# apple/ml-mdm

Measured on AMD Instinct MI355X. Metric: denoise-steps/sec, whole job = N x optimizer steps/s at per-GPU batch 64 (train fwd+bwd+optimizer, cc12m_64x64 U-Net), higher is better.
Workload: dtype bf16; 1 GPU; unet64 train step, per-GPU batch 64, global batch 64; global_batch=64, parallelism=dp1, settle_steps=15

## Files before the change

### include/mdm_hip_ext.h

```cpp
#ifndef MDM_HIP_EXT_H_
#define MDM_HIP_EXT_H_
#ifdef __cplusplus
extern "C" {
#endif

int mdm_attn_cross_bias(const void* qkv, const void* kvc, const float* mask, const float* bias, int bias_ld,
                        const void* base, int base_ld, void* out, int B, int L, int S, int H, int d, int dtype,
                        void* stream);

int mdm_freeu_plan(int N, int H, int W, int C1, int C2, int dtype, int structure, size_t* ws_bytes);
int mdm_freeu_stats(const void* h, const void* r, void* ws, size_t ws_bytes, int N, int H, int W, int C1, int C2,
                    int structure, int dtype, void* stream);
int mdm_freeu_apply(const void* h, const void* r, const void* ws, size_t ws_bytes, void* out, int N, int H, int W, int C1,
                    int C2, float b, float s, int structure, int dtype, void* stream);

int mdm_cfg_plan(int B, size_t chw, int rescale_on, size_t* ws_bytes);
int mdm_cfg_stats(const float* x_t, const float* pred, const float* pred_uncond, const float* gamma, const float* run_prev,
                  float* run_out, const float* run_gate, const float* w_gate, float momentum, int rescale_on, void* ws,
                  size_t ws_bytes, int B, size_t chw, int pred_type, void* stream);
int mdm_cfg_combine(const float* x_t, const float* pred, const float* pred_uncond, const float* gamma, const float* run,
                    const float* w_gate, const void* ws, size_t ws_bytes, float* out, float guidance, float eta,
                    float norm_threshold, float rescale, float image_scale, int B, size_t chw, int pred_type, void* stream);

int mdm_tiles_gather(const float* x, float* out, int B, int C, int H, int W, int h, int w, int sy, int sx, int reps,
                     void* stream);
int mdm_tiles_merge(const float* p, float* out, int R, int C, int H, int W, int h, int w, int sy, int sx, int blend,
                    void* stream);

int mdm_abs_quantile_plan(int B, size_t n, size_t* ws_bytes);
int mdm_abs_quantile(const float* x, void* ws, size_t ws_bytes, int B, size_t n, float q, float cmin, float cmax, float* thr,
                     float* stats, void* stream);

int mdm_t5_attn_fwd_lse(const void* qkv, const int* seq_start, const int* pos, const float* bias_table, void* out, float* lse,
                        int B, int T, int S, int max_len, int H, int d, int dtype, void* stream);
int mdm_t5_attn_bwd(const void* qkv, const void* out, const float* lse, const void* dout, const int* seq_start, const int* pos,
                    const float* bias_table, void* dqkv, int B, int T, int S, int max_len, int H, int d, int dtype,
                    void* stream);
int mdm_t5_gated_gelu_bwd(const void* u, const void* dy, void* du, int T, int F, int dtype, void* stream);
int mdm_t5_rms_bwd(const float* x, const float* ln_w, const void* dh, float* dx, void* dx_lo, int T, int D, float eps,
                   int dtype, void* stream);
int mdm_t5_final_rms_bwd(const float* x, const void* delta, const float* ln_w, const float* dout, const int* flat, float* dx,
                         void* dx_lo, int T, int D, float eps, int dtype, void* stream);
int mdm_t5_embed_rms_slots(const int* ids, const float* table, const int* slot_of_id, const float* learned, const float* ln_w,
                           float* x, void* h, int T, int D, int vocab, int n_ids, int P, float eps, int dtype, void* stream);
int mdm_t5_embed_bwd(const float* dx0, const int* slot_start, const int* tokens, float* dlearned, int P, int D, int n, int T,
                     void* stream);

int mdm_sampler_step_sa(const float* x_t, const float* pred, const float* pred_uncond, float guidance, const float* gamma,
                        const float* gamma_last, const float* gamma_h0, const float* gamma_h1, const float* gate,
                        const float* thr, const float* noise, const unsigned long long* rng_state, int rng_stream, float* h0,
                        float* h1, float* psum, float* x0_out, float* x_last_out, int B, size_t chw, int pred_type, int clip,
                        float image_scale, int max_predictor, int max_corrector, void* stream);

#ifdef __cplusplus
}
#endif
#endif
```

### ml-mdm_amd/csrc/gemm_conv.hip

```cpp
#include <stdio.h>
#include <stdlib.h>

#include <type_traits>
#include <utility>

#include "common.hpp"
#include "conv_args.hpp"

namespace mdm {



__device__ __forceinline__ void load4(const float* p, float (&o)[4]) {
  const f32x4 t = *reinterpret_cast<const f32x4*>(p);
  o[0] = t[0]; o[1] = t[1]; o[2] = t[2]; o[3] = t[3];
}
__device__ __forceinline__ void load4(const bf16* p, float (&o)[4]) {
  const bf16x4 t = *reinterpret_cast<const bf16x4*>(p);
  o[0] = (float)t[0]; o[1] = (float)t[1]; o[2] = (float)t[2]; o[3] = (float)t[3];
}

__device__ __attribute__((aligned(16))) uint4 g_zero_page[4] = {};


// ... 1165 lines not shown
#define MDM_BLDS(rs, lds_off, voff, soff)                                                                   \
  __builtin_amdgcn_raw_ptr_buffer_load_lds(rs, (__attribute__((address_space(3))) void*)(lds_off), 16, voff, soff, 0, 0)
#define MDM_WG_TILE_STATE(it_)                                                                              \
  const bool more_ = (it_) < nt;                                                                            \
  const auto rsA = __builtin_amdgcn_make_buffer_rsrc(a_base, 0, more_ ? a_bytes : 0u, 0x00020000);         \
  const auto rsB = __builtin_amdgcn_make_buffer_rsrc(b_base, 0, more_ ? b_bytes : 0u, 0x00020000);         \
  const int mb_ = (mt_begin + (it_)) * BKM;                                                                 \
  const int a_soff = mb_ * p.Cout * 2, b_soff = mb_ * p.Cin * 2;
#define MDM_WG_PIECE(stage, q)                                                                              \
  {                                                                                                         \
    constexpr int j_ = (q) >> 1;                                                                            \
    const int m_ = mb_ + j_ * RPP + srow;                                                                   \
    bool v_ = m_ < p.M;                                                                                     \
    if (((q) & 1) == 0) {                                                                                   \
      MDM_BLDS(rsA, (stage) + j_ * (RPP * ROWB) + wave_lds, v_ ? a_vo[j_] : INVALID, a_soff);               \
    } else {                                                                                                \
      if (MODE == MODE_3x3) {                                                                               \
        const int ow_ = m_ & (p.W - 1), oh_ = (m_ >> logW) & (p.H - 1);                                     \
        v_ = v_ && (unsigned)(oh_ + kh - 1) < (unsigned)p.H && (unsigned)(ow_ + kw - 1) < (unsigned)p.W;    \
      }                                                                                                     \
      MDM_BLDS(rsB, (stage) + A_BYTES + j_ * (RPP * ROWB) + wave_lds, v_ ? b_vo[j_] : INVALID, b_soff);     \
    }                                                                                                       \
  }

  f32x4 acc[MT][NT];
#pragma unroll
  for (int i = 0; i < MT; ++i)
#pragma unroll
    for (int j = 0; j < NT; ++j) acc[i][j] = f32x4{0.f, 0.f, 0.f, 0.f};
  const int bias_k0 = (MODE == MODE_3x3 && p.skip_cout > 0) ? (((n0 / p.skip_cout) >> 1) * 3 + ((n0 / p.skip_cout) & 1)) * p.Cin : 0;
  constexpr int BR = MT / NWN;
  const int wn_s = __builtin_amdgcn_readfirstlane(wn);
  const int bias_share = p.groups > 0 ? 1 : p.bias_share;
  const int kt_rel = k0 >= bias_k0 ? (k0 - bias_k0) / BN : bias_share;
  const bool bias_blk = (p.groups > 0 ? gr.bout[grp] != nullptr : p.bslab != nullptr) && kt_rel < bias_share;
  const int bias_chunk = (nt + bias_share - 1) / bias_share;
  const int bias_b0 = bias_blk ? min(kt_rel * bias_chunk, nt) : nt;
  const int bias_b1 = bias_blk ? min(bias_b0 + bias_chunk, nt) : nt;

  unsigned fa[MT], fb[NT];
  {
    const unsigned smem_base = (unsigned)(size_t)(__attribute__((address_space(3))) char*)smem;
    const int r0 = quad * 8 + (l16 >> 2);
    const int fsw = (l16 >> 2) | ((quad & 1) << 2);
#pragma unroll
    for (int c = 0; c < MT; ++c) fa[c] = smem_base + r0 * ROWB + (((wm * MT + c) ^ fsw) << 5) + ((l16 & 3) << 3);
#pragma unroll
    for (int c = 0; c < NT; ++c) fb[c] = smem_base + A_BYTES + r0 * ROWB + (((wn * NT + c) ^ fsw) << 5) + ((l16 & 3) << 3);
  }

  if (nt > 0) {
    {
      MDM_WG_TILE_STATE(0);
      MDM_WG_PIECE(smem, 0); MDM_WG_PIECE(smem, 1); MDM_WG_PIECE(smem, 2); MDM_WG_PIECE(smem, 3);
      MDM_WG_PIECE(smem, 4); MDM_WG_PIECE(smem, 5); MDM_WG_PIECE(smem, 6); MDM_WG_PIECE(smem, 7);
    }
    {
      MDM_WG_TILE_STATE(1);
      MDM_WG_PIECE(smem + STAGE, 0); MDM_WG_PIECE(smem + STAGE, 1); MDM_WG_PIECE(smem + STAGE, 2); MDM_WG_PIECE(smem + STAGE, 3);
      MDM_WG_PIECE(smem + STAGE, 4); MDM_WG_PIECE(smem + STAGE, 5); MDM_WG_PIECE(smem + STAGE, 6); MDM_WG_PIECE(smem + STAGE, 7);
    }
    asm volatile("s_waitcnt vmcnt(0)" ::: "memory");
    __syncthreads();
    u32x2 ra[MT][2], rb0[NT][2], rb1[NT][2];
#pragma unroll
    for (int c = 0; c < NT; ++c) MDM_TR2(rb0[c][0], rb0[c][1], fb[c], 0);
#pragma unroll
    for (int c = 0; c < MT; ++c) MDM_TR2(ra[c][0], ra[c][1], fa[c], 0);
    __builtin_amdgcn_sched_barrier(0);

#define MDM_WG_ITER(BIAS)                                                                                   \
    {                                                                                                       \
      const unsigned so = (unsigned)((it & 1) * STAGE), sn = (unsigned)(((it + 1) & 1) * STAGE);            \
                                                                     \
      _Pragma("unroll") for (int c = 0; c < NT; ++c) { const unsigned ad = fb[c] + so; MDM_TR2(rb1[c][0], rb1[c][1], ad, KS1); } \
      Frag<T> bq[NT];                                                                                       \
      _Pragma("unroll") for (int i = 0; i < MT; ++i) {                                                      \
        if (i == 0) {                                                                                       \
          asm volatile("s_waitcnt lgkmcnt(%8)"                                                              \
                       : "+v"(rb0[0][0]), "+v"(rb0[0][1]), "+v"(rb0[1][0]), "+v"(rb0[1][1]), "+v"(rb0[2][0]), \
                         "+v"(rb0[2][1]), "+v"(rb0[3][0]), "+v"(rb0[3][1])                                  \
                       : "n"(WAITN) : "memory");                                                            \
          _Pragma("unroll") for (int j = 0; j < NT; ++j) bq[j] = frag_of(rb0[j][0], rb0[j][1]);             \
        }                                                                                                   \
        asm volatile("s_waitcnt lgkmcnt(%2)" : "+v"(ra[i][0]), "+v"(ra[i][1]) : "n"(WAITN) : "memory");     \
        const Frag<T> aq = frag_of(ra[i][0], ra[i][1]);                                                     \
        _Pragma("unroll") for (int j = 0; j < NT; ++j) mma16(acc[i][j], bq[j], aq);                         \
        if (BIAS && i / BR == wn_s) bsum[i % BR] = frag_sum_guarded(aq, bsum[i % BR]);                      \
        { const unsigned ad = fa[i] + so; MDM_TR2(ra[i][0], ra[i][1], ad, KS1); }                           \
        __builtin_amdgcn_sched_barrier(0);                                                                  \
      }                                                                                                     \
                                        \
      asm volatile("s_waitcnt vmcnt(0) lgkmcnt(0)" ::: "memory");                                           \
      __builtin_amdgcn_s_barrier();                                                                         \
      __builtin_amdgcn_sched_barrier(0);                                                                    \
              \
      MDM_WG_TILE_STATE(it + 2);                                                                            \
      char* const dst = smem + so;                                                                          \
      _Pragma("unroll") for (int c = 0; c < NT; ++c) { const unsigned ad = fb[c] + sn; MDM_TR2(rb0[c][0], rb0[c][1], ad, 0); } \
      _Pragma("unroll") for (int j = 0; j < NT; ++j) bq[j] = frag_of(rb1[j][0], rb1[j][1]);                 \
      _Pragma("unroll") for (int i = 0; i < MT; ++i) {                                                      \
        const Frag<T> aq = frag_of(ra[i][0], ra[i][1]);                                                     \
        _Pragma("unroll") for (int j = 0; j < NT; ++j) mma16(acc[i][j], bq[j], aq);                         \
        if (BIAS && i / BR == wn_s) bsum[i % BR] = frag_sum_guarded(aq, bsum[i % BR]);                      \
        if (MT == 8) { MDM_WG_PIECE_RT(dst, i) } else { MDM_WG_PIECE_RT(dst, 2 * i) MDM_WG_PIECE_RT(dst, 2 * i + 1) } \
        { const unsigned ad = fa[i] + sn; MDM_TR2(ra[i][0], ra[i][1], ad, 0); }                             \
        __builtin_amdgcn_sched_barrier(0);                                                                  \
      }                                                                                                     \
    }
#define MDM_WG_PIECE_RT(stage, q)                                                                           \
    switch (q) {                                                                                            \
      case 0: MDM_WG_PIECE(stage, 0) break; case 1: MDM_WG_PIECE(stage, 1) break;                           \
      case 2: MDM_WG_PIECE(stage, 2) break; case 3: MDM_WG_PIECE(stage, 3) break;                           \
      case 4: MDM_WG_PIECE(stage, 4) break; case 5: MDM_WG_PIECE(stage, 5) break;                           \
      case 6: MDM_WG_PIECE(stage, 6) break; default: MDM_WG_PIECE(stage, 7) break;                          \
    }
    int it = 0;
    float bsum[BR];
    for (; it < bias_b0; ++it) MDM_WG_ITER(false)
#pragma unroll
    for (int i = 0; i < BR; ++i) bsum[i] = 0.f;
    for (; it < bias_b1; ++it) MDM_WG_ITER(true)
    if (bias_blk) {
#pragma unroll
      for (int r = 0; r < BR; ++r) {
        float v = bsum[r];
        v += __shfl_xor(v, 16, 64);
        v += __shfl_xor(v, 32, 64);
        const int n = n0 + wm * TM + (wn * BR + r) * 16 + l16;
        if (quad == 0 && n < p.Cout) {
          if (p.groups > 0) gr.bout[grp][n] += v;
          else p.bslab[((size_t)split * bias_share + kt_rel) * p.Cout + n] = v;
        }
      }
    }
    for (; it < nt; ++it) MDM_WG_ITER(false)
    asm volatile("s_waitcnt vmcnt(0) lgkmcnt(0)" ::: "memory");
#undef MDM_WG_PIECE_RT
#undef MDM_WG_ITER
  } else if (bias_blk && p.groups == 0 && quad == 0) {
#pragma unroll
    for (int r = 0; r < BR; ++r) {
      const int n = n0 + wm * TM + (wn * BR + r) * 16 + l16;
      if (n < p.Cout) p.bslab[((size_t)split * bias_share + kt_rel) * p.Cout + n] = 0.f;
    }
  }
#undef MDM_WG_PIECE
#undef MDM_WG_TILE_STATE
#undef MDM_BLDS

  if (bias_blk && p.groups == 0 && split == 0 && kt_rel == 0 && n0 == 0 && tid == 0)
    reinterpret_cast<int*>(p.bslab - WG_BHDR)[0] = bias_share;
  const bool direct = p.groups > 0;
  float* __restrict__ S = direct ? gr.out[grp] : p.slab + (size_t)split * p.Cout * p.K;
  const bool vec_ok = (p.K & 3) == 0;
  if (!direct) {
#pragma unroll
    for (int i = 0; i < MT; ++i) {
      const int n = n0 + wm * TM + i * 16 + l16;
      if (n >= p.Cout) continue;
#pragma unroll
      for (int j = 0; j < NT; ++j) {
        const int k = k0 + wn * TN + j * 16 + quad * 4;
        if (k >= p.K) continue;
        float* o = S + (size_t)n * p.K + k;
        if (vec_ok) {
          *reinterpret_cast<f32x4*>(o) = acc[i][j];
        } else {
#pragma unroll
          for (int e = 0; e < 4; ++e) if (k + e < p.K) o[e] = acc[i][j][e];
        }
      }
    }
  } else if (vec_ok && n0 + BM <= p.Cout && k0 + BN <= p.K) {
    float* const o0 = S + (size_t)(n0 + wm * TM + l16) * p.K + k0 + wn * TN + quad * 4;
    f32x4 old[2][NT];
#pragma unroll
    for (int j = 0; j < NT; ++j) old[0][j] = *reinterpret_cast<const f32x4*>(o0 + j * 16);
#pragma unroll
    for (int i = 0; i < MT; ++i) {
      if (i + 1 < MT) {
#pragma unroll
        for (int j = 0; j < NT; ++j) old[(i + 1) & 1][j] = *reinterpret_cast<const f32x4*>(o0 + (size_t)(i + 1) * 16 * p.K + j * 16);
      }
#pragma unroll
      for (int j = 0; j < NT; ++j) *reinterpret_cast<f32x4*>(o0 + (size_t)i * 16 * p.K + j * 16) = old[i & 1][j] + acc[i][j];
    }
  } else {
#pragma unroll
    for (int i = 0; i < MT; ++i) {
      const int n = n0 + wm * TM + i * 16 + l16;
      if (n >= p.Cout) continue;
#pragma unroll
      for (int j = 0; j < NT; ++j) {
        const int k = k0 + wn * TN + j * 16 + quad * 4;
        if (k >= p.K) continue;
        float* o = S + (size_t)n * p.K + k;
#pragma unroll
        for (int e = 0; e < 4; ++e) if (k + e < p.K) o[e] += acc[i][j][e];
      }
    }
  }
#endif
}
#undef MDM_TR2

template <int NT>
__device__ __forceinline__ void wgrad_bias_reduce(const float* __restrict__ bslab, float* __restrict__ dbias, int splits,
                                                  int Cout, int accumulate, int blk, float* lds) {
  constexpr int G = NT / 32;
  const int tid = threadIdx.x, c = tid & 31, g = tid >> 5;
  const int rows = splits * reinterpret_cast<const int*>(bslab - WG_BHDR)[0];
  const int o = blk * 32 + c;
  float s0 = 0.f, s1 = 0.f, s2 = 0.f, s3 = 0.f;
  if (o < Cout) {
    const float* src = bslab + o;
    int r = g;
    for (; r + 3 * G < rows; r += 4 * G) {
      s0 += src[(size_t)r * Cout];
      s1 += src[(size_t)(r + G) * Cout];
      s2 += src[(size_t)(r + 2 * G) * Cout];
      s3 += src[(size_t)(r + 3 * G) * Cout];
    }
    for (; r < rows; r += G) s0 += src[(size_t)r * Cout];
  }
  lds[tid] = (s0 + s1) + (s2 + s3);
  __syncthreads();
  if (g == 0 && o < Cout) {
    float s = lds[c];
#pragma unroll
    for (int q = 1; q < G; ++q) s += lds[q * 32 + c];
    dbias[o] = accumulate ? dbias[o] + s : s;
  }
}

__global__ __launch_bounds__(192) void wgrad_reduce_kernel(const float* __restrict__ slab, float* __restrict__ dw,
                                                           const float* __restrict__ bslab, float* __restrict__ dbias,
                                                           int splits, int Cout, int Cin, int taps, int accumulate,
                                                           int bblocks) {
  __shared__ float tile[64 * 9 + 4];
  const int tid = threadIdx.x;
  if ((int)blockIdx.x < bblocks) {
    wgrad_bias_reduce<192>(bslab, dbias, splits, Cout, accumulate, (int)blockIdx.x, tile);
    return;
  }
  const int wb = (int)blockIdx.x - bblocks;
  const int iblocks = (Cin + 63) / 64;
  const int o = wb / iblocks, i0 = (wb - o * iblocks) * 64;
  const int ni = min(64, Cin - i0);
  const size_t total = (size_t)Cout * Cin * taps;
  const int K = Cin * taps;
  const int per_o = taps * 16;
  if (tid < per_o) {
    const int tp = tid >> 4, i4 = (tid & 15) * 4;
    f32x4 acc[8];
#pragma unroll
    for (int u = 0; u < 8; ++u) acc[u] = f32x4{0.f, 0.f, 0.f, 0.f};
    if (i4 < ni) {
      const float* src = slab + (size_t)o * K + (size_t)tp * Cin + i0 + i4;
      int sp = 0;
      for (; sp + 8 <= splits; sp += 8) {
#pragma unroll
        for (int u = 0; u < 8; ++u) acc[u] += *reinterpret_cast<const f32x4*>(src + (size_t)(sp + u) * total);
      }
      for (; sp < splits; ++sp) acc[0] += *reinterpret_cast<const f32x4*>(src + (size_t)sp * total);
    }
    const f32x4 s4 = ((acc[0] + acc[1]) + (acc[2] + acc[3])) + ((acc[4] + acc[5]) + (acc[6] + acc[7]));
#pragma unroll
    for (int q = 0; q < 4; ++q) tile[(i4 + q) * taps + tp] = s4[q];
  }
  __syncthreads();
  const int run = ni * taps;
  float* const dst = dw + ((size_t)o * Cin + i0) * taps;
  for (int r = tid; r < run; r += 192) dst[r] = accumulate ? dst[r] + tile[r] : tile[r];
}

__global__ __launch_bounds__(256) void wgrad_reduce_flat_kernel(const float* __restrict__ slab, float* __restrict__ dw,
                                                                const float* __restrict__ bslab,
                                                                float* __restrict__ dbias, int splits, int Cout,
                                                                size_t total, int accumulate, int wblocks, int bblocks) {
  if ((int)blockIdx.x < bblocks) {
    __shared__ float part[256];
    wgrad_bias_reduce<256>(bslab, dbias, splits, Cout, accumulate, (int)blockIdx.x, part);
    return;
  }
  const size_t n4 = total / 4;
  const f32x4* s4 = reinterpret_cast<const f32x4*>(slab);
  f32x4* d4 = reinterpret_cast<f32x4*>(dw);
  for (size_t i = (size_t)(blockIdx.x - bblocks) * 256 + threadIdx.x; i < n4; i += (size_t)wblocks * 256) {
    f32x4 a0 = s4[i], a1 = {0.f, 0.f, 0.f, 0.f}, a2 = a1, a3 = a1;
    int sp = 1;
    for (; sp + 4 <= splits; sp += 4) {
      a0 += s4[(size_t)sp * n4 + i];
      a1 += s4[(size_t)(sp + 1) * n4 + i];
      a2 += s4[(size_t)(sp + 2) * n4 + i];
      a3 += s4[(size_t)(sp + 3) * n4 + i];
    }
    for (; sp < splits; ++sp) a0 += s4[(size_t)sp * n4 + i];
    const f32x4 a = (a0 + a1) + (a2 + a3);
    d4[i] = accumulate ? d4[i] + a : a;
  }
}

template <typename T>
__global__ void pack_weight_kernel(const float* __restrict__ w, T* __restrict__ wf, T* __restrict__ wd,
                                   int Cout, int Cin, int taps, int Cin_pad, int Cout_pad, int kbf, int kbd) {
  const size_t Kf = (size_t)taps * Cin_pad, Kd = (size_t)taps * Cout_pad;
  const size_t total_f = (size_t)Cout * Kf;
  const size_t total_d = wd ? (size_t)Cin * Kd : 0;
  for (size_t idx = (size_t)blockIdx.x * blockDim.x + threadIdx.x; idx < total_f + total_d;
       idx += (size_t)gridDim.x * blockDim.x) {
    if (idx < total_f) {
      const int o = (int)(idx / Kf);
      const int kpos = (int)(idx - (size_t)o * Kf);
      int tp, i;
      if (kbf) { const int cb = kpos / (taps * kbf), r = kpos - cb * taps * kbf; tp = r / kbf; i = cb * kbf + (r - tp * kbf); }
      else { tp = kpos / Cin_pad; i = kpos - tp * Cin_pad; }
      wf[idx] = from_f32<T>(i < Cin ? w[((size_t)o * Cin + i) * taps + tp] : 0.f);
    } else {
      const size_t d = idx - total_f;
      const int i = (int)(d / Kd);
      const int kpos = (int)(d - (size_t)i * Kd);
      int tp, o;
      if (kbd) { const int ob = kpos / (taps * kbd), r = kpos - ob * taps * kbd; tp = r / kbd; o = ob * kbd + (r - tp * kbd); }
      else { tp = kpos / Cout_pad; o = kpos - tp * Cout_pad; }
      wd[d] = from_f32<T>(o < Cout ? w[((size_t)o * Cin + i) * taps + (taps - 1 - tp)] : 0.f);
    }
  }
}

template <typename T, int TAPS>
__global__ __launch_bounds__(256) void pack_weight_tiled_kernel(const float* __restrict__ w, T* __restrict__ wf,
                                                                T* __restrict__ wd, int Cout, int Cin, int kbf,
                                                                int kbd) {
  __shared__ float tile[32][32 * TAPS + 1];
  const int ib = blockIdx.x * 32, ob = blockIdx.y * 32;
  const int tid = threadIdx.x;
  for (int e = tid; e < 32 * 32 * TAPS; e += 256) {
    const int ol = e / (32 * TAPS), r = e - ol * (32 * TAPS);
    tile[ol][r] = w[((size_t)(ob + ol) * Cin + ib) * TAPS + r];
  }
  __syncthreads();
  const size_t Kf = (size_t)TAPS * Cin, Kd = (size_t)TAPS * Cout;
  for (int e = tid; e < 32 * TAPS * 32; e += 256) {
    const int il = e & 31, rest = e >> 5;
    const int tp = rest % TAPS, ol = rest / TAPS;
    const int i = ib + il;
    const size_t kpos = kbf ? (size_t)(i / kbf) * TAPS * kbf + (size_t)tp * kbf + (i % kbf) : (size_t)tp * Cin + i;
    wf[(size_t)(ob + ol) * Kf + kpos] = from_f32<T>(tile[ol][il * TAPS + tp]);
  }
  if (wd) {
    for (int e = tid; e < 32 * TAPS * 32; e += 256) {
      const int ol = e & 31, rest = e >> 5;
      const int tp = rest % TAPS, il = rest / TAPS;
      const int o = ob + ol;
      const size_t kpos = kbd ? (size_t)(o / kbd) * TAPS * kbd + (size_t)tp * kbd + (o % kbd) : (size_t)tp * Cout + o;
      wd[(size_t)(ib + il) * Kd + kpos] = from_f32<T>(tile[ol][il * TAPS + (TAPS - 1 - tp)]);
    }
  }
}

struct PackDesc {
  const float* w;
  void* wf;
  void* wd;
  int Cout, Cin, taps, kbf, kbd;
  int first_block;
};

template <typename T, int TAPS>
__device__ __forceinline__ void pack_brick(const PackDesc& d, int brick, float (*tile)[32 * 9 + 1]) {
  constexpr int V = 16 / (int)sizeof(T), NV = 32 / V;
  const int ibn = d.Cin / 32;
  const int ib = (brick % ibn) * 32, ob = (brick / ibn) * 32;
  const int tid = threadIdx.x;
  const int Cin = d.Cin, Cout = d.Cout;
  for (int e = tid; e < 32 * 8 * TAPS; e += 256) {
    const int ol = e / (8 * TAPS), q = e - ol * (8 * TAPS);
    const f32x4 v = *reinterpret_cast<const f32x4*>(d.w + ((size_t)(ob + ol) * Cin + ib) * TAPS + q * 4);
#pragma unroll
    for (int j = 0; j < 4; ++j) tile[ol][q * 4 + j] = v[j];
  }
  __syncthreads();
  const size_t Kf = (size_t)TAPS * Cin, Kd = (size_t)TAPS * Cout;
  T* wf = reinterpret_cast<T*>(d.wf);
  T* wd = reinterpret_cast<T*>(d.wd);
  for (int e = tid; e < 32 * TAPS * NV; e += 256) {
    const int iv = e % NV, rest = e / NV;
    const int tp = rest % TAPS, ol = rest / TAPS;
    const int i = ib + iv * V;
    const size_t kpos = d.kbf ? (size_t)(i / d.kbf) * TAPS * d.kbf + (size_t)tp * d.kbf + (i % d.kbf) : (size_t)tp * Cin + i;
    T out[V];
#pragma unroll
    for (int j = 0; j < V; ++j) out[j] = from_f32<T>(tile[ol][(iv * V + j) * TAPS + tp]);
    *reinterpret_cast<uint4*>(wf + (size_t)(ob + ol) * Kf + kpos) = *reinterpret_cast<const uint4*>(out);
  }
  if (wd) {
    for (int e = tid; e < 32 * TAPS * NV; e += 256) {
      const int ov = e % NV, rest = e / NV;
      const int tp = rest % TAPS, il = rest / TAPS;
      const int o = ob + ov * V;
      const size_t kpos = d.kbd ? (size_t)(o / d.kbd) * TAPS * d.kbd + (size_t)tp * d.kbd + (o % d.kbd) : (size_t)tp * Cout + o;
      T out[V];
#pragma unroll
      for (int j = 0; j < V; ++j) out[j] = from_f32<T>(tile[ov * V + j][il * TAPS + (TAPS - 1 - tp)]);
      *reinterpret_cast<uint4*>(wd + (size_t)(ib + il) * Kd + kpos) = *reinterpret_cast<const uint4*>(out);
    }
  }
}

template <typename T>
__global__ __launch_bounds__(256) void pack_weights_multi_kernel(const PackDesc* __restrict__ table, int n) {
  __shared__ float tile[32][32 * 9 + 1];
  int lo = 0, hi = n - 1;
  const int b = blockIdx.x;
  while (lo < hi) {
    const int mid = (lo + hi + 1) >> 1;
    if (table[mid].first_block <= b) lo = mid; else hi = mid - 1;
  }
  const PackDesc d = table[lo];
  if (d.taps == 9) pack_brick<T, 9>(d, b - d.first_block, tile);
  else pack_brick<T, 1>(d, b - d.first_block, tile);
}

template <typename T>
__global__ __launch_bounds__(256) void colsum_partial_kernel(const T* __restrict__ x, float* __restrict__ part,
                                                             int M, int C, int rows_per_slab) {
  constexpr int EPV = Tr<T>::EPV;
  __shared__ float red[32][8][8];
  const int tid = threadIdx.x, tc = tid & 7, tr = tid >> 3;
  const int chunk = blockIdx.x * 8 + tc;
  const bool cok = chunk * EPV < C;
  const int m_begin = blockIdx.y * rows_per_slab, m_end = min(M, m_begin + rows_per_slab);
  float s[EPV];
#pragma unroll
  for (int e = 0; e < EPV; ++e) s[e] = 0.f;
  if (cok) {
    for (int m = m_begin + tr; m < m_end; m += 32) {
      Chunk<T> ch;
      ch.load(x + (size_t)m * C + (size_t)chunk * EPV);
#pragma unroll
      for (int e = 0; e < EPV; ++e) s[e] += ch.v[e];
    }
  }
#pragma unroll
  for (int e = 0; e < EPV; ++e) red[tr][tc][e] = s[e];
  __syncthreads();
  if (tid < 8 * EPV) {
    const int c = tid / EPV, e = tid - c * EPV;
    float a = 0.f;
#pragma unroll 8
    for (int r = 0; r < 32; ++r) a += red[r][c][e];
    const int ch = (blockIdx.x * 8 + c) * EPV + e;
    if (ch < C) part[(size_t)blockIdx.y * C + ch] = a;
  }
}
__global__ void colsum_final_kernel(const float* __restrict__ part, float* __restrict__ out, int nslabs, int C,
                                    int accumulate) {
  const int c = blockIdx.x * blockDim.x + threadIdx.x;
  if (c >= C) return;
  float s = 0.f;
  for (int b = 0; b < nslabs; ++b) s += part[(size_t)b * C + c];
  out[c] = accumulate ? out[c] + s : s;
}

}

using namespace mdm;

template <typename T>
__global__ __launch_bounds__(256) void splitk_epilogue_kernel(const float* __restrict__ part, int ksplit, size_t mc,
                                                              int Cout, const float* __restrict__ bias,
                                                              const T* __restrict__ res, const T* __restrict__ aux,
                                                              T* __restrict__ y, T* __restrict__ ypre, int act) {
  const size_t idx = ((size_t)blockIdx.x * 256 + threadIdx.x) * 4;
  if (idx >= mc) return;
  f32x4 s = *reinterpret_cast<const f32x4*>(part + idx);
  for (int sp = 1; sp < ksplit; ++sp) s += *reinterpret_cast<const f32x4*>(part + (size_t)sp * mc + idx);
  const int n = (int)(idx % (size_t)Cout);
  if (bias) s += *reinterpret_cast<const f32x4*>(bias + n);
  float v[4];
#pragma unroll
  for (int e = 0; e < 4; ++e) v[e] = to_f32(from_f32<T>(s[e]));
  if (act == 1) {
    if (ypre) {
      if constexpr (sizeof(T) == 2 && kFfnAuxByte) {
        *reinterpret_cast<unsigned*>(reinterpret_cast<unsigned char*>(ypre) + idx) = DGeluCode::enc4(v);
      } else {
#pragma unroll
        for (int e = 0; e < 4; ++e) ypre[idx + e] = from_f32<T>(v[e]);
      }
    }
    gelu_vec<T, 4>(v);
  } else if (act == 2) {
    if constexpr (sizeof(T) == 2 && kFfnAuxByte) {
      float g[4];
      DGeluCode::dec4(*reinterpret_cast<const unsigned*>(reinterpret_cast<const unsigned char*>(aux) + idx), g);
#pragma unroll
      for (int e = 0; e < 4; ++e) v[e] *= g[e];
    } else {
      float ax[4];
#pragma unroll
      for (int e = 0; e < 4; ++e) ax[e] = to_f32(aux[idx + e]);
      mul_dgelu_vec<T, 4>(v, ax);
    }
  }
  if (res) {
#pragma unroll
    for (int e = 0; e < 4; ++e) v[e] += to_f32(res[idx + e]);
  }
#pragma unroll
  for (int e = 0; e < 4; ++e) y[idx + e] = from_f32<T>(v[e]);
}

__device__ __forceinline__ bool up_tap_in(int ph, int a, int kh) {
  return ph == 0 ? (a == 0 ? kh == 0 : kh >= 1) : (a == 0 ? kh <= 1 : kh == 2);
}
__global__ __launch_bounds__(256) void upconv_pack_kernel(const float* __restrict__ w, bf16* __restrict__ w_ph,
                                                          int Cout, int Cin) {
  const int idx = blockIdx.x * 256 + threadIdx.x;
  if (idx >= Cout * Cin) return;
  const int co = idx / Cin, ci = idx - co * Cin;
  float t[9];
#pragma unroll
  for (int k = 0; k < 9; ++k) t[k] = w[(size_t)idx * 9 + k];
#pragma unroll
  for (int ph = 0; ph < 2; ++ph)
#pragma unroll
    for (int pw = 0; pw < 2; ++pw)
#pragma unroll
      for (int a = 0; a < 2; ++a)
#pragma unroll
        for (int b = 0; b < 2; ++b) {
          float v = 0.f;
#pragma unroll
          for (int kh = 0; kh < 3; ++kh)
#pragma unroll
            for (int kw = 0; kw < 3; ++kw)
              if (up_tap_in(ph, a, kh) && up_tap_in(pw, b, kw)) v += t[kh * 3 + kw];
          const int phase = ph * 2 + pw;
          w_ph[((size_t)(phase * Cout + co) * (Cin >> 6) + (ci >> 6)) * 256 + (a * 2 + b) * 64 + (ci & 63)] = (bf16)v;
        }
}
__global__ __launch_bounds__(256) void upconv_pack_t_kernel(const float* __restrict__ w, bf16* __restrict__ w_t, int Cout,
                                                            int Cin) {
  __shared__ float t[64][16 * 9 + 1];
  const int cib = Cin / 16;
  const int co0 = ((int)blockIdx.x / cib) * 64, ci0 = ((int)blockIdx.x % cib) * 16;
  const int tid = threadIdx.x;
  for (int e = tid; e < 64 * 144; e += 256) {
    const int co_l = e / 144, r = e - co_l * 144;
    t[co_l][r] = w[((size_t)(co0 + co_l) * Cin + ci0) * 9 + r];
  }
  __syncthreads();
  for (int e = tid; e < 4 * 16 * 256; e += 256) {
    const int co_l = e & 63, j = (e >> 6) & 3, ci_l = (e >> 8) & 15, phase = e >> 12;
    const int ph = phase >> 1, pw = phase & 1, a = 1 - (j >> 1), b = 1 - (j & 1);
    float v = 0.f;
#pragma unroll
    for (int kh = 0; kh < 3; ++kh)
#pragma unroll
      for (int kw = 0; kw < 3; ++kw)
        if (up_tap_in(ph, a, kh) && up_tap_in(pw, b, kw)) v += t[co_l][ci_l * 9 + kh * 3 + kw];
    w_t[(((size_t)(ci0 + ci_l) * 4 + phase) * (Cout >> 6) + (co0 >> 6)) * 256 + j * 64 + co_l] = (bf16)v;
  }
}

__global__ __launch_bounds__(256) void s2dgrad_pack_kernel(const float* __restrict__ w, bf16* __restrict__ w_sel, int Cout,
                                                           int Cin) {
  __shared__ float t[64][16 * 9 + 1];
  const int cib = Cin / 16;
  const int co0 = ((int)blockIdx.x / cib) * 64, ci0 = ((int)blockIdx.x % cib) * 16;
  const int tid = threadIdx.x;
  for (int e = tid; e < 64 * 144; e += 256) {
    const int co_l = e / 144, r = e - co_l * 144;
    t[co_l][r] = w[((size_t)(co0 + co_l) * Cin + ci0) * 9 + r];
  }
  __syncthreads();
  for (int e = tid; e < 4 * 16 * 256; e += 256) {
    const int co_l = e & 63, j = (e >> 6) & 3, ci_l = (e >> 8) & 15, phase = e >> 12;
    const int ph = phase >> 1, pw = phase & 1, dh = j >> 1, dw = j & 1;
    const int kh = ph == 0 ? (dh == 0 ? 1 : -1) : (dh == 0 ? 2 : 0);
    const int kw = pw == 0 ? (dw == 0 ? 1 : -1) : (dw == 0 ? 2 : 0);
    const float v = (kh >= 0 && kw >= 0) ? t[co_l][ci_l * 9 + kh * 3 + kw] : 0.f;
    w_sel[(((size_t)(phase * Cin + ci0 + ci_l) * (Cout >> 6) + (co0 >> 6)) * 4 + j) * 64 + co_l] = (bf16)v;
  }
}

__global__ __launch_bounds__(256) void upconv_wfold_kernel(const float* __restrict__ dwb, float* __restrict__ dw, int Cout,
                                                           int Cin, int accumulate) {
  const int idx = blockIdx.x * 256 + threadIdx.x;
  if (idx >= Cout * Cin) return;
  const int co = idx / Cin, ci = idx - co * Cin;
  float o[9];
#pragma unroll
  for (int k = 0; k < 9; ++k) o[k] = 0.f;
#pragma unroll
  for (int ph = 0; ph < 2; ++ph)
#pragma unroll
    for (int pw = 0; pw < 2; ++pw)
#pragma unroll
      for (int a = 0; a < 2; ++a)
#pragma unroll
        for (int b = 0; b < 2; ++b) {
          const float g = dwb[((size_t)((ph * 2 + pw) * Cout + co) * Cin + ci) * 9 + (ph + a) * 3 + (pw + b)];
#pragma unroll
          for (int kh = 0; kh < 3; ++kh)
#pragma unroll
            for (int kw = 0; kw < 3; ++kw)
              if (up_tap_in(ph, a, kh) && up_tap_in(pw, b, kw)) o[kh * 3 + kw] += g;
        }
#pragma unroll
  for (int k = 0; k < 9; ++k) {
    float* d = dw + (size_t)idx * 9 + k;
    *d = accumulate ? *d + o[k] : o[k];
  }
}

__global__ __launch_bounds__(256) void upconv_bfold_kernel(const float* __restrict__ db4, float* __restrict__ db, int Cout,
                                                           int accumulate) {
  const int co = blockIdx.x * 256 + threadIdx.x;
  if (co >= Cout) return;
  const float v = (db4[co] + db4[Cout + co]) + (db4[2 * Cout + co] + db4[3 * Cout + co]);
  db[co] = accumulate ? db[co] + v : v;
}

static int g_dev_flags = 0;
static inline ConvArgs with_dev_flags(const ConvArgs& a) { ConvArgs b = a; b.dev_flags = g_dev_flags; return b; }
static thread_local char g_last_gemm[96] = "";
extern "C" const char* mdm_last_gemm_kernel(void) { return g_last_gemm; }
#define MDM_NOTE_KERNEL(...) snprintf(g_last_gemm, sizeof(g_last_gemm), __VA_ARGS__)
template <typename T, int BM, int BN, int WM, int WN, int MODE, int SPLIT = 0>
static int launch_conv_cfg(const ConvArgs& a_, hipStream_t st) {
  const ConvArgs a = with_dev_flags(a_);
  constexpr int smem = 2 * (BM + BN) * 128;
  auto kern = conv_gemm_kernel<T, BM, BN, WM, WN, MODE, SPLIT>;
  ensure_dynamic_lds(kern, smem);
  const int tiles = ((a.M + BM - 1) / BM) * ((a.Cout + BN - 1) / BN);
  hipLaunchKernelGGL(kern, dim3(tiles), dim3(WM * WN * 64), smem, st, a);
  MDM_NOTE_KERNEL("conv_gemm_kernel<%s, %d, %d, %d, %d, %d>", sizeof(T) == 2 ? "bf16" : (SPLIT == 2 ? "float (bf16x3, weight planes)" : (SPLIT ? "float (bf16x3)" : "float")), BM, BN, WM, WN, MODE);
  MDM_LAUNCH_STATUS();
}

template <int BM, int BN, int WM, int WN, int MODE>
static int launch_conv_bl(const ConvArgs& a_, hipStream_t st) {
  const ConvArgs a = with_dev_flags(a_);
  constexpr int smem = 2 * (BM + BN) * 128;
  auto kern = conv_gemm_bl_kernel<BM, BN, WM, WN, MODE>;
  ensure_dynamic_lds(kern, smem);
  const int tiles = ((a.M + BM - 1) / BM) * ((a.Cout + BN - 1) / BN);
  if constexpr (BM == 128 && BN == 128) {
    if (tiles <= device_cus()) {
      auto kern4 = conv_gemm_bl_kernel<BM, BN, WM, WN, MODE, false, false, false, 4>;
      ensure_dynamic_lds(kern4, 2 * smem);
      hipLaunchKernelGGL(kern4, dim3(tiles), dim3(WM * WN * 64), 2 * smem, st, a, NoConvGroup{});
      MDM_NOTE_KERNEL("conv_gemm_bl_kernel<%d, %d, %d, %d, %d, 4 stages>", BM, BN, WM, WN, MODE);
      MDM_LAUNCH_STATUS();
    }
  }
  const int resident = device_cus() * (WM * WN == 4 ? 2 : 1);
  hipLaunchKernelGGL(kern, dim3(tiles < resident ? tiles : resident), dim3(WM * WN * 64), smem, st, a, NoConvGroup{});
  MDM_NOTE_KERNEL("conv_gemm_bl_kernel<%d, %d, %d, %d, %d>", BM, BN, WM, WN, MODE);
  MDM_LAUNCH_STATUS();
}

template <int BM, int BN, int WM, int WN>
static int launch_conv_bl_sel4(const ConvArgs& a_, hipStream_t st) {
  const ConvArgs a = with_dev_flags(a_);
  constexpr int smem = 2 * (BM + BN) * 128;
  auto kern = conv_gemm_bl_kernel<BM, BN, WM, WN, MODE_3x3, false, false, true>;
  ensure_dynamic_lds(kern, smem);
  const int tiles = ((a.M + BM - 1) / BM) * ((a.Cout + BN - 1) / BN);
  const int resident = device_cus() * (WM * WN == 4 ? 2 : 1);
  hipLaunchKernelGGL(kern, dim3(tiles < resident ? tiles : resident), dim3(WM * WN * 64), smem, st, a, NoConvGroup{});
  MDM_NOTE_KERNEL("conv_gemm_bl_kernel<%d, %d, %d, %d, %d, sel4>", BM, BN, WM, WN, MODE_3x3);
  MDM_LAUNCH_STATUS();
}

template <int BM, int BN, int WM, int WN>
static int launch_conv_bl_grouped(const ConvArgs& a_, const ConvGroup& gr, hipStream_t st) {
  const ConvArgs a = with_dev_flags(a_);
  constexpr int smem = 2 * (BM + BN) * 128;
  auto kern = conv_gemm_bl_kernel<BM, BN, WM, WN, MODE_1x1, true>;
  ensure_dynamic_lds(kern, smem);
  const int tiles = ((a.M + BM - 1) / BM) * ((a.Cout + BN - 1) / BN) * a.groups;
  const int resident = device_cus() * (WM * WN == 4 ? 2 : 1);
  hipLaunchKernelGGL(kern, dim3(tiles < resident ? tiles : resident), dim3(WM * WN * 64), smem, st, a, gr);
  MDM_NOTE_KERNEL("conv_gemm_bl_kernel<%d, %d, %d, %d, %d, grouped>", BM, BN, WM, WN, MODE_1x1);
  MDM_LAUNCH_STATUS();
}

template <typename T, int MODE>
static bool conv_bl_ok(const ConvArgs& a) {
  if (sizeof(T) != 2 || MODE == MODE_3x3_T2) return false;
  if (a.K % 64 != 0 || (MODE == MODE_3x3 && a.kblk == 0)) return false;
  const size_t lim = 0x7F000000u;
  const size_t bias = MODE == MODE_3x3 ? (size_t)(a.W + 1) * a.Cin * 2 : 0;
  if ((size_t)a.N * a.H * a.W * a.Cin * 2 + bias > lim || (size_t)a.Cout * a.K * 2 > lim) return false;
  return 2 * bias + (size_t)a.K * 2 < 0x00F00000u;
}

static int conv_ksplit(int M, int Cout, int K, int dtype) {
  if (dtype != DT_BF16 || K % 64 != 0 || Cout % 8 != 0 || Cout <= 64) return 1;
  constexpr int fill = 80, minkt = 6, minsave = 16;
  const long tiles = (long)((M + 127) / 128) * ((Cout + 127) / 128);
  const int nt = K / 64, cus = device_cus();
  if (tiles * 100 > (long)fill * 2 * cus || nt < 2 * minkt) return 1;
  const int per_cu = M <= 2048 ? 1 : 2;
  long sp = ((long)per_cu * cus) / tiles;
  if (sp > nt / minkt) sp = nt / minkt;
  if (sp > 16) sp = 16;
  if (sp < 2 || nt - (nt + sp - 1) / sp < minsave) return 1;
  return (int)sp;
}

extern "C" int mdm_conv_fwd_plan(int M, int Cout, int K, int dtype, int* splits, size_t* ws_bytes) {
  MDM_CHECK_ARG(splits && ws_bytes && M > 0 && Cout > 0 && K > 0);
  *splits = conv_ksplit(M, Cout, K, dtype);
  *ws_bytes = *splits > 1 ? (size_t)*splits * M * Cout * sizeof(float) : 0;
  return 0;
}

template <int MODE>
static int launch_conv_bl_splitk(ConvArgs a, int splits, float* ws, hipStream_t st) {
// ... 417 lines not shown
  const wg_s16x4 b = __builtin_amdgcn_ds_read_tr16_b64_v4i16((__attribute__((address_space(3))) wg_s16x4*)(p + second));
  typedef __attribute__((ext_vector_type(8))) short s16x8;
  s16x8 v = {a[0], a[1], a[2], a[3], b[0], b[1], b[2], b[3]};
  Frag<bf16> f;
  f.v = __builtin_bit_cast(bf16x8, v);
  return f;
}

template <int CIN, int TAPS, int TH>
__global__ __launch_bounds__(512, 1) void wgrad_direct_kernel(WgDirectArgs p) {
  constexpr int COUT = 64, TW = 32, HALO = TAPS == 9 ? 1 : 0;
  constexpr int TWH = TW + 2 * HALO, THH = TH + 2 * HALO;
  constexpr int XCH = CIN / 8, DCH = COUT / 8;
  constexpr int PX = wgd_pitch(CIN * 2), PD = wgd_pitch(COUT * 2);
  constexpr int K = TAPS * CIN;
  constexpr int NBW = K / 16 / 4;
  static_assert((K / 16) % 4 == 0, "K columns split over 4 waves");
  constexpr int XROW = TWH * XCH, XCHUNKS = THH * XROW, DCHUNKS = TH * TW * DCH;
  constexpr int NXL = (XCHUNKS + 511) / 512, NDL = (DCHUNKS + 511) / 512;
  extern __shared__ __attribute__((aligned(16))) char dsm[];
  char* const xs = dsm;
  char* const ys = dsm + THH * TWH * PX;
  const int tid = threadIdx.x, lane = tid & 63, wid = tid >> 6;
  const int l15 = lane & 15, quad = lane >> 4;
  const int mw = wid >> 2, nw = wid & 3;

  const int trow = 8 * quad + (l15 >> 2), tseg = (l15 & 3) * 8;
  int y_off[2], x_off[NBW];
#pragma unroll
  for (int mi = 0; mi < 2; ++mi) y_off[mi] = trow * PD + (mw * 2 + mi) * 32 + tseg;
#pragma unroll
  for (int nb = 0; nb < NBW; ++nb) {
    const int nbg = nw * NBW + nb, tap = nbg / (CIN / 16), cb = nbg - tap * (CIN / 16);
    const int dy_ = TAPS == 9 ? tap / 3 : 0, dx_ = TAPS == 9 ? tap % 3 : 0;
    x_off[nb] = (dy_ * TWH + dx_ + trow) * PX + cb * 32 + tseg;
  }

  f32x4 acc[NBW][2];
#pragma unroll
  for (int nb = 0; nb < NBW; ++nb)
#pragma unroll
    for (int mi = 0; mi < 2; ++mi) acc[nb][mi] = f32x4{0.f, 0.f, 0.f, 0.f};
  float bsum[2] = {0.f, 0.f};
  const bool do_bias = p.bslab != nullptr && nw == 0;

  uint4 prex[NXL], prey[NDL];
  auto issue = [&](int tile) {
    const int tx = tile % p.tiles_x, ty = (tile / p.tiles_x) % p.tiles_y, n = tile / (p.tiles_x * p.tiles_y);
    const int gx0 = tx * TW - HALO, gy0 = ty * TH - HALO;
    const bf16* xn = p.x + (size_t)n * p.H * p.W * CIN;
#pragma unroll
    for (int i = 0; i < NXL; ++i) {
      const int c = tid + 512 * i;
      const int row = c / XROW, col = c - row * XROW, px = col / XCH, ch = col - px * XCH;
      const int gy = gy0 + row, gx = gx0 + px;
      prex[i] = uint4{0u, 0u, 0u, 0u};
      if (c < XCHUNKS && (unsigned)gy < (unsigned)p.H && (unsigned)gx < (unsigned)p.W)
        prex[i] = *reinterpret_cast<const uint4*>(xn + ((size_t)gy * p.W + gx) * CIN + ch * 8);
    }
    const bf16* yn = p.dy + (((size_t)n * p.H + ty * TH) * p.W + tx * TW) * COUT;
#pragma unroll
    for (int i = 0; i < NDL; ++i) {
      const int c = tid + 512 * i;
      const int row = c / (TW * DCH), col = c - row * (TW * DCH);
      prey[i] = uint4{0u, 0u, 0u, 0u};
      if (c < DCHUNKS) prey[i] = *reinterpret_cast<const uint4*>(yn + (size_t)row * p.W * COUT + col * 8);
    }
  };
  if ((int)blockIdx.x < p.tiles) issue(blockIdx.x);
  for (int tile = blockIdx.x; tile < p.tiles; tile += gridDim.x) {
#pragma unroll
    for (int i = 0; i < NXL; ++i) {
      const int c = tid + 512 * i;
      const int row = c / XROW, col = c - row * XROW, px = col / XCH, ch = col - px * XCH;
      if (c < XCHUNKS) *reinterpret_cast<uint4*>(xs + (row * TWH + px) * PX + ch * 16) = prex[i];
    }
#pragma unroll
    for (int i = 0; i < NDL; ++i) {
      const int c = tid + 512 * i;
      const int pix = c / DCH, ch = c - pix * DCH;
      if (c < DCHUNKS) *reinterpret_cast<uint4*>(ys + pix * PD + ch * 16) = prey[i];
    }
    __syncthreads();
    if (tile + (int)gridDim.x < p.tiles) issue(tile + gridDim.x);
#pragma unroll 2
    for (int r = 0; r < TH; ++r) {
      Frag<bf16> yf[2];
#pragma unroll
      for (int mi = 0; mi < 2; ++mi) yf[mi] = wgd_tr2(ys + r * (TW * PD) + y_off[mi], 4 * PD);
      if (do_bias) {
#pragma unroll
        for (int mi = 0; mi < 2; ++mi) bsum[mi] = frag_sum(yf[mi], bsum[mi]);
      }
#pragma unroll
      for (int nb = 0; nb < NBW; ++nb) {
        const Frag<bf16> xf = wgd_tr2(xs + r * (TWH * PX) + x_off[nb], 4 * PX);
#pragma unroll
        for (int mi = 0; mi < 2; ++mi) mma16(acc[nb][mi], xf, yf[mi]);
      }
    }
    __syncthreads();
  }
  float* const S = p.slab + (size_t)blockIdx.x * COUT * K;
#pragma unroll
  for (int nb = 0; nb < NBW; ++nb)
#pragma unroll
    for (int mi = 0; mi < 2; ++mi)
      *reinterpret_cast<f32x4*>(S + (size_t)((mw * 2 + mi) * 16 + l15) * K + (nw * NBW + nb) * 16 + quad * 4) = acc[nb][mi];
  if (do_bias) {
#pragma unroll
    for (int mi = 0; mi < 2; ++mi) {
      float v = bsum[mi];
      v += __shfl_xor(v, 16, 64);
      v += __shfl_xor(v, 32, 64);
      if (quad == 0) p.bslab[(size_t)blockIdx.x * COUT + (mw * 2 + mi) * 16 + l15] = v;
    }
  }
  if (p.bslab != nullptr && blockIdx.x == 0 && tid == 0) reinterpret_cast<int*>(p.bslab - WG_BHDR)[0] = 1;
}

constexpr int WGD_SLABS = 256;
static int wgrad_direct_slabs(int M, int Cout, int K, int dtype) {
  if (g_no_wgrad_direct || dtype != DT_BF16 || Cout != 64 || M < 262144) return 0;
  return (K == 576 || K == 128 || K == 192) ? WGD_SLABS : 0;
}
static bool wgrad_direct_ok(const WgradArgs& a, int ksize) {
  if (a.stride != 1 || a.Ho != a.H || a.Wo != a.W || a.Cout != 64 || a.skip_cout) return false;
  if (!(ksize == 3 && a.Cin == 64)) return false;
  if (((uintptr_t)a.x & 15) || ((uintptr_t)a.dy & 15)) return false;
  if (a.H % 8 != 0 || a.W % 32 != 0) return false;
  return (long)a.N * (a.H / 8) * (a.W / 32) >= WGD_SLABS;
}
template <int CIN, int TAPS, int TH>
static int launch_wgrad_direct(const WgradArgs& a, hipStream_t st) {
  constexpr int HALO = TAPS == 9 ? 1 : 0;
  constexpr int smem = (TH + 2 * HALO) * (32 + 2 * HALO) * wgd_pitch(CIN * 2) + TH * 32 * wgd_pitch(128);
  static_assert(smem <= 160 * 1024, "LDS");
  auto kern = wgrad_direct_kernel<CIN, TAPS, TH>;
  ensure_dynamic_lds(kern, smem);
  WgDirectArgs d;
  d.x = (const bf16*)a.x; d.dy = (const bf16*)a.dy; d.slab = a.slab; d.bslab = a.bslab;
  d.N = a.N; d.H = a.H; d.W = a.W; d.tiles_x = d.W / 32; d.tiles_y = d.H / TH; d.tiles = d.tiles_x * d.tiles_y * d.N;
  hipLaunchKernelGGL(kern, dim3(WGD_SLABS), dim3(512), smem, st, d);
  MDM_NOTE_KERNEL("wgrad_direct_kernel<%d, %d, %d>", CIN, TAPS, TH);
  MDM_LAUNCH_STATUS();
}

static void wgrad_choose(int M, int Cout, int K, int dtype, int* te_out, int* splits_out) {
  if (const int slabs = wgrad_direct_slabs(M, Cout, K, dtype)) { *te_out = 128; *splits_out = slabs; return; }
  const int bkm = dtype == DT_F32 ? 32 : 64;
  const int mt_total = (M + bkm - 1) / bkm;
  double best = 1e30;
  int best_te = 128, best_s = 1;
  const int forced = wgrad_forced_tile(Cout, K, dtype);
  for (int te = 128; te <= 256; te += 128) {
    if (te == 256 && !(dtype == DT_BF16 && Cout >= 192 && K >= 192)) continue;
    if (forced && te != forced) continue;
    const int tiles = ((Cout + te - 1) / te) * ((K + te - 1) / te);
    const int slots = te == 256 ? 256 : 512;
    const double t_tile = (te == 256 ? 1.7 : 1.06) * (dtype == DT_F32 ? 8.0 : 1.0), t_fix = te == 256 ? 12.0 : 5.0;
    const int smax = mt_total < 64 ? mt_total : 64;
    for (int sp = 1; sp <= smax; ++sp) {
      const int per = (mt_total + sp - 1) / sp;
      if ((mt_total + per - 1) / per != sp) continue;
      const long blocks = (long)tiles * sp;
      const double rounds = (double)((blocks + slots - 1) / slots);
      const double cost = rounds * (per * t_tile + t_fix) + sp * (double)Cout * K * 4.0 / 5.0e6 + (sp > 1 ? 4.0 : 0.0);
      if (cost < best) { best = cost; best_te = te; best_s = sp; }
    }
  }
  *te_out = best_te;
  *splits_out = best_s;
}

static int wgrad_tile(int M, int Cout, int K, int dtype) {
  int te, sp;
  wgrad_choose(M, Cout, K, dtype, &te, &sp);
  return te;
}

extern "C" int mdm_conv_wgrad_tile(int M, int Cout, int K, int dtype) { return wgrad_tile(M, Cout, K, dtype); }

extern "C" int mdm_conv_wgrad_plan(int M, int Cout, int K, int dtype, int* splits_out, size_t* ws_bytes) {
  MDM_CHECK_ARG(splits_out && ws_bytes);
  int te, splits;
  wgrad_choose(M, Cout, K, dtype, &te, &splits);
  *splits_out = splits;
  const int brows = splits * WG_BSHARE > 64 ? splits * WG_BSHARE : 64;
  *ws_bytes = ((size_t)splits * Cout * K + WG_BHDR + (size_t)brows * Cout) * sizeof(float);
  return 0;
}

extern "C" int mdm_colsum(const void* x, float* out, float* ws, int M, int C, int accumulate, int dtype, void* stream);

static bool wgrad_bl_ok(const WgradArgs& a, int ksize) {
  if (ksize == 3) {
    if (a.stride != 1 || a.Ho != a.H || a.Wo != a.W) return false;
    if ((a.H & (a.H - 1)) || (a.W & (a.W - 1))) return false;
  }
  const size_t lim = 0x7F000000u;
  const size_t bias = ksize == 3 ? (size_t)(a.W + 1) * a.Cin * 2 : 0;
  return (size_t)a.M * a.Cout * 2 <= lim && (size_t)a.N * a.H * a.W * a.Cin * 2 + bias <= lim;
}

static int conv_wgrad_impl(const void* x, const void* dy, int want_bias, float* ws, int N, int H, int W, int Cin,
                           int Ho, int Wo, int Cout, int ksize, int stride, int dtype, int skip_cout, void* stream) {
  MDM_CHECK_ARG(x && dy && ws);
  MDM_CHECK_ARG(ksize == 1 || ksize == 3);
  MDM_CHECK_ARG(dtype == DT_F32 || dtype == DT_BF16);
  const int epv = dtype == DT_F32 ? 4 : 8;
  MDM_CHECK_ARG(Cin % epv == 0 && Cout % epv == 0);
  WgradArgs a = {};
  a.x = x; a.dy = dy; a.slab = ws; a.skip_cout = skip_cout;
  a.N = N; a.H = H; a.W = W; a.Cin = Cin; a.Ho = Ho; a.Wo = Wo; a.Cout = Cout; a.stride = stride;
  a.M = N * Ho * Wo; a.K = ksize * ksize * Cin; a.groups = 0;
  size_t wsb;
  int rc = mdm_conv_wgrad_plan(a.M, Cout, a.K, dtype, &a.splits, &wsb);
  if (rc) return rc;
  const int bkm = dtype == DT_F32 ? 32 : 64;
  const int mt_total = (a.M + bkm - 1) / bkm;
  a.mtiles_per_split = (mt_total + a.splits - 1) / a.splits;
  float* const bias_ws = ws + (size_t)a.splits * Cout * a.K;
  a.bslab = (want_bias && dtype == DT_BF16) ? bias_ws + WG_BHDR : nullptr;
  const int te = wgrad_tile(a.M, Cout, a.K, dtype);
  const int tiles = ((Cout + te - 1) / te) * ((a.K + te - 1) / te);
  {
    const int kt = skip_cout > 0 ? Cin / te : (a.K + te - 1) / te;
    a.bias_share = kt < WG_BSHARE ? (kt < 1 ? 1 : kt) : WG_BSHARE;
  }
  hipStream_t st = reinterpret_cast<hipStream_t>(stream);
  if (wgrad_direct_slabs(a.M, Cout, a.K, dtype) && wgrad_direct_ok(a, ksize)) {
    return launch_wgrad_direct<64, 9, 8>(a, st);
  }
  constexpr int smem = 4 * 128 * 128, smem_big = 4 * 64 * 512;
  ensure_dynamic_lds(conv_wgrad_kernel<float, MODE_1x1>, smem);
  ensure_dynamic_lds(conv_wgrad_kernel<float, MODE_3x3>, smem);
  ensure_dynamic_lds(conv_wgrad_tr_kernel<MODE_1x1, 0>, smem);
  ensure_dynamic_lds(conv_wgrad_tr_kernel<MODE_3x3, 0>, smem);
  ensure_dynamic_lds(conv_wgrad_tr_kernel<MODE_1x1, 1>, smem_big);
  ensure_dynamic_lds(conv_wgrad_tr_kernel<MODE_3x3, 1>, smem_big);
  ensure_dynamic_lds(conv_wgrad_bl_kernel<MODE_1x1, 0>, smem);
  ensure_dynamic_lds(conv_wgrad_bl_kernel<MODE_3x3, 0>, smem);
  ensure_dynamic_lds(conv_wgrad_bl_kernel<MODE_1x1, 1>, smem_big);
  ensure_dynamic_lds(conv_wgrad_bl_kernel<MODE_3x3, 1>, smem_big);
  dim3 grid(tiles * a.splits);
  const int mode = ksize == 1 ? MODE_1x1 : MODE_3x3;
  if (dtype == DT_F32) MDM_NOTE_KERNEL("conv_wgrad_kernel<float, %d>", mode);
  else if (wgrad_bl_ok(a, ksize)) MDM_NOTE_KERNEL("conv_wgrad_bl_kernel<%d, %d>", mode, te == 256 ? 1 : 0);
  else MDM_NOTE_KERNEL("conv_wgrad_tr_kernel<%d, %d>", mode, te == 256 ? 1 : 0);
  if (dtype == DT_F32) {
    if (ksize == 1) hipLaunchKernelGGL((conv_wgrad_kernel<float, MODE_1x1>), grid, dim3(256), smem, st, a);
    else hipLaunchKernelGGL((conv_wgrad_kernel<float, MODE_3x3>), grid, dim3(256), smem, st, a);
  } else if (wgrad_bl_ok(a, ksize)) {
    if (te == 256) {
      if (ksize == 1) hipLaunchKernelGGL((conv_wgrad_bl_kernel<MODE_1x1, 1>), grid, dim3(512), smem_big, st, a, WgradGroup{});
      else hipLaunchKernelGGL((conv_wgrad_bl_kernel<MODE_3x3, 1>), grid, dim3(512), smem_big, st, a, WgradGroup{});
    } else {
      if (ksize == 1) hipLaunchKernelGGL((conv_wgrad_bl_kernel<MODE_1x1, 0>), grid, dim3(256), smem, st, a, WgradGroup{});
      else hipLaunchKernelGGL((conv_wgrad_bl_kernel<MODE_3x3, 0>), grid, dim3(256), smem, st, a, WgradGroup{});
    }
  } else if (te == 256) {
    if (ksize == 1) hipLaunchKernelGGL((conv_wgrad_tr_kernel<MODE_1x1, 1>), grid, dim3(512), smem_big, st, a);
    else hipLaunchKernelGGL((conv_wgrad_tr_kernel<MODE_3x3, 1>), grid, dim3(512), smem_big, st, a);
  } else {
    if (ksize == 1) hipLaunchKernelGGL((conv_wgrad_tr_kernel<MODE_1x1, 0>), grid, dim3(256), smem, st, a);
    else hipLaunchKernelGGL((conv_wgrad_tr_kernel<MODE_3x3, 0>), grid, dim3(256), smem, st, a);
  }
  MDM_LAUNCH_STATUS();
}

extern "C" int mdm_conv_wgrad(const void* x, const void* dy, int want_bias, float* ws, int N, int H, int W, int Cin,
                              int Ho, int Wo, int Cout, int ksize, int stride, int dtype, void* stream) {
  return conv_wgrad_impl(x, dy, want_bias, ws, N, H, W, Cin, Ho, Wo, Cout, ksize, stride, dtype, 0, stream);
}

extern "C" int mdm_conv_wgrad_blocked(const void* x, const void* dyb, int want_bias, float* ws, int N, int H, int W, int Cin,
                                      int Cout, int dtype, void* stream) {
  MDM_CHECK_ARG(dtype == DT_BF16 && Cin % 256 == 0 && Cout % 256 == 0);
  MDM_CHECK_ARG((H & (H - 1)) == 0 && (W & (W - 1)) == 0);
  return conv_wgrad_impl(x, dyb, want_bias, ws, N, H, W, Cin, H, W, 4 * Cout, 3, 1, dtype, Cout, stream);
}

static int wgrad_group_tile(int M, int Cout, int K, int groups) {
  if (groups < 2 || groups > WG_MAXG || M < 4096) return 0;
  if (const int forced = wgrad_forced_tile(Cout, K, DT_BF16)) return forced;
  const long t256 = (long)((Cout + 255) / 256) * ((K + 255) / 256) * groups;
  const long t128 = (long)((Cout + 127) / 128) * ((K + 127) / 128) * groups;
  const int cus = device_cus();
  if (Cout >= 192 && K >= 192) {
    const double eff = (double)t256 / (double)(((t256 + cus - 1) / cus) * cus);
    if (t256 >= (long)(0.7 * cus) && eff >= 0.7) return 256;
  }
  const double eff = (double)t128 / (double)(((t128 + 2 * cus - 1) / (2 * cus)) * 2 * cus);
  if (t128 >= (long)(1.4 * cus) && eff >= 0.7) return 128;
  return 0;
}

extern "C" int mdm_conv_wgrad_group_plan(int M, int Cout, int K, int dtype, int groups, int* tile_out) {
  MDM_CHECK_ARG(tile_out);
  *tile_out = dtype == DT_BF16 ? wgrad_group_tile(M, Cout, K, groups) : 0;
  return 0;
}

extern "C" int mdm_conv_wgrad_grouped(const void* const* x, const void* const* dy, float* const* dw,
                                      float* const* dbias, int groups, int M, int Cin, int Cout, int dtype,
                                      void* stream) {
  MDM_CHECK_ARG(x && dy && dw && groups >= 1 && groups <= WG_MAXG);
  MDM_CHECK_ARG(dtype == DT_BF16 && Cin % 8 == 0 && Cout % 8 == 0 && M > 0);
  WgradArgs a = {};
  a.N = M; a.H = 1; a.W = 1; a.Cin = Cin; a.Ho = 1; a.Wo = 1; a.Cout = Cout; a.stride = 1;
  a.M = M; a.K = Cin; a.splits = 1; a.groups = groups;
  a.mtiles_per_split = (M + 63) / 64;
  MDM_CHECK_ARG(wgrad_bl_ok(a, 1));
  WgradGroup gr = {};
  for (int g = 0; g < groups; ++g) {
    MDM_CHECK_ARG(x[g] && dy[g] && dw[g]);
    gr.x[g] = x[g]; gr.dy[g] = dy[g]; gr.out[g] = dw[g]; gr.bout[g] = dbias ? dbias[g] : nullptr;
  }
  int te = wgrad_group_tile(M, Cout, Cin, groups);
  if (!te) te = wgrad_forced_tile(Cout, Cin, DT_BF16);
  if (!te) te = (Cout >= 192 && Cin >= 192) ? 256 : 128;
  const int tiles = ((Cout + te - 1) / te) * ((Cin + te - 1) / te);
  hipStream_t st = reinterpret_cast<hipStream_t>(stream);
  constexpr int smem = 4 * 128 * 128, smem_big = 4 * 64 * 512;
  if (te == 256) {
    ensure_dynamic_lds(conv_wgrad_bl_kernel<MODE_1x1, 1>, smem_big);
    hipLaunchKernelGGL((conv_wgrad_bl_kernel<MODE_1x1, 1>), dim3(tiles * groups), dim3(512), smem_big, st, a, gr);
  } else {
    ensure_dynamic_lds(conv_wgrad_bl_kernel<MODE_1x1, 0>, smem);
    hipLaunchKernelGGL((conv_wgrad_bl_kernel<MODE_1x1, 0>), dim3(tiles * groups), dim3(256), smem, st, a, gr);
  }
  MDM_NOTE_KERNEL("conv_wgrad_bl_kernel<%d, %d>", MODE_1x1, te == 256 ? 1 : 0);
  MDM_LAUNCH_STATUS();
}

extern "C" int mdm_conv_wgrad_reduce(const float* ws, float* dw_oihw, float* dbias, const void* dy, int M, int Cin,
                                     int Cout, int ksize, int accumulate, int dtype, void* stream) {
  MDM_CHECK_ARG(ws && dw_oihw && (ksize == 1 || ksize == 3));
  const int K = ksize * ksize * Cin;
  int splits; size_t wsb;
  int rc = mdm_conv_wgrad_plan(M, Cout, K, dtype, &splits, &wsb);
  if (rc) return rc;
  hipStream_t st = reinterpret_cast<hipStream_t>(stream);
  float* const bias_ws = const_cast<float*>(ws) + (size_t)splits * Cout * K;
  const float* bslab = (dbias && dtype == DT_BF16) ? bias_ws + WG_BHDR : nullptr;
  const int bblocks = bslab ? (Cout + 31) / 32 : 0;
  if (ksize == 1) {
    const size_t total = (size_t)Cout * Cin;
    const int wblocks = (int)((total / 4 + 255) / 256 > 2048 ? 2048 : (total / 4 + 255) / 256);
    hipLaunchKernelGGL(wgrad_reduce_flat_kernel, dim3(wblocks + bblocks), dim3(256), 0, st, ws, dw_oihw, bslab, dbias,
                       splits, Cout, total, accumulate, wblocks, bblocks);
  } else {
    const int wblocks = Cout * ((Cin + 63) / 64);
    hipLaunchKernelGGL(wgrad_reduce_kernel, dim3(wblocks + bblocks), dim3(192), 0, st, ws, dw_oihw, bslab, dbias,
                       splits, Cout, Cin, ksize * ksize, accumulate, bblocks);
  }
  if (dbias && !bslab) {
    MDM_CHECK_ARG(dy);
    return mdm_colsum(dy, dbias, bias_ws, M, Cout, accumulate, dtype, stream);
  }
  MDM_LAUNCH_STATUS();
}

extern "C" int mdm_pack_weight(const float* w_oihw, void* w_fwd, void* w_dgrad, int Cout, int Cin, int ksize,
                               int Cin_pad, int Cout_pad, int kblock_fwd, int kblock_dgrad, int dtype,
                               void* stream) {
  MDM_CHECK_ARG(w_oihw && w_fwd);
  MDM_CHECK_ARG(ksize == 1 || ksize == 3);
  MDM_CHECK_ARG(Cin_pad >= Cin && Cout_pad >= Cout);
  MDM_CHECK_ARG(kblock_fwd == 0 || (ksize == 3 && Cin_pad % kblock_fwd == 0));
  MDM_CHECK_ARG(kblock_dgrad == 0 || (ksize == 3 && Cout_pad % kblock_dgrad == 0));
  const int taps = ksize * ksize;
  const size_t total = (size_t)Cout * taps * Cin_pad + (w_dgrad ? (size_t)Cin * taps * Cout_pad : 0);
  const int nb = (int)((total + 255) / 256 > 8192 ? 8192 : (total + 255) / 256);
  hipStream_t st = reinterpret_cast<hipStream_t>(stream);
  if (Cin_pad == Cin && Cout_pad == Cout && Cin % 32 == 0 && Cout % 32 == 0) {
    dim3 grid(Cin / 32, Cout / 32);
#define MDM_PACK_TILED(TT, TAPS)                                                                               \
  hipLaunchKernelGGL((pack_weight_tiled_kernel<TT, TAPS>), grid, dim3(256), 0, st, w_oihw, (TT*)w_fwd, (TT*)w_dgrad, \
                     Cout, Cin, kblock_fwd, kblock_dgrad)
    if (dtype == DT_F32) { if (taps == 9) MDM_PACK_TILED(float, 9); else MDM_PACK_TILED(float, 1); }
    else if (dtype == DT_BF16) { if (taps == 9) MDM_PACK_TILED(bf16, 9); else MDM_PACK_TILED(bf16, 1); }
    else MDM_CHECK_ARG(false);
#undef MDM_PACK_TILED
    MDM_LAUNCH_STATUS();
  }
  if (dtype == DT_F32)
    hipLaunchKernelGGL(pack_weight_kernel<float>, dim3(nb), dim3(256), 0, st, w_oihw, (float*)w_fwd, (float*)w_dgrad, Cout, Cin, taps, Cin_pad, Cout_pad, kblock_fwd, kblock_dgrad);
  else if (dtype == DT_BF16)
    hipLaunchKernelGGL(pack_weight_kernel<bf16>, dim3(nb), dim3(256), 0, st, w_oihw, (bf16*)w_fwd, (bf16*)w_dgrad, Cout, Cin, taps, Cin_pad, Cout_pad, kblock_fwd, kblock_dgrad);
  else MDM_CHECK_ARG(false);
  MDM_LAUNCH_STATUS();
}

extern "C" int mdm_pack_weights_multi(const void* table, int n, int total_blocks, int dtype, void* stream) {
  MDM_CHECK_ARG(table && n > 0 && total_blocks > 0);
  static_assert(sizeof(PackDesc) == 48, "descriptor layout is part of the ABI");
  hipStream_t st = reinterpret_cast<hipStream_t>(stream);
  if (dtype == DT_F32) hipLaunchKernelGGL(pack_weights_multi_kernel<float>, dim3(total_blocks), dim3(256), 0, st, (const PackDesc*)table, n);
  else if (dtype == DT_BF16) hipLaunchKernelGGL(pack_weights_multi_kernel<bf16>, dim3(total_blocks), dim3(256), 0, st, (const PackDesc*)table, n);
  else MDM_CHECK_ARG(false);
  MDM_LAUNCH_STATUS();
}

static inline int colsum_slabs(int M, int C, int epv) {
  const int groups = (C + 8 * epv - 1) / (8 * epv);
  int slabs = (1024 + groups - 1) / groups;
  const int max_slabs = (M + 63) / 64;
  if (slabs > max_slabs) slabs = max_slabs;
  if (slabs > 64) slabs = 64;
  if (slabs < 1) slabs = 1;
  return slabs;
}

extern "C" int mdm_colsum_plan(int M, int C, int* nblocks, size_t* ws_bytes) {
  MDM_CHECK_ARG(nblocks && ws_bytes);
  const int slabs = colsum_slabs(M, C, 4);
  *nblocks = slabs;
  *ws_bytes = (size_t)64 * C * sizeof(float);
  return 0;
}

extern "C" int mdm_colsum(const void* x, float* out, float* ws, int M, int C, int accumulate, int dtype,
                          void* stream) {
  MDM_CHECK_ARG(x && out && ws);
  MDM_CHECK_ARG(dtype == DT_F32 || dtype == DT_BF16);
  const int epv = dtype == DT_F32 ? 4 : 8;
  MDM_CHECK_ARG(C % epv == 0);
  const int slabs = colsum_slabs(M, C, epv);
  const int rps = (M + slabs - 1) / slabs;
  const int groups = (C + 8 * epv - 1) / (8 * epv);
  hipStream_t st = reinterpret_cast<hipStream_t>(stream);
  if (dtype == DT_F32)
    hipLaunchKernelGGL(colsum_partial_kernel<float>, dim3(groups, slabs), dim3(256), 0, st, (const float*)x, ws, M, C, rps);
  else
    hipLaunchKernelGGL(colsum_partial_kernel<bf16>, dim3(groups, slabs), dim3(256), 0, st, (const bf16*)x, ws, M, C, rps);
  hipLaunchKernelGGL(colsum_final_kernel, dim3((C + 255) / 256), dim3(256), 0, st, ws, out, slabs, C, accumulate);
  MDM_LAUNCH_STATUS();
}
```

### ml-mdm_amd/mdm_hip/distributed.py

```python
import os
from datetime import timedelta

import torch
import torch.distributed as dist


def get_rank() -> int:
    return dist.get_rank() if dist.is_available() and dist.is_initialized() else 0


def get_world_size() -> int:
    return dist.get_world_size() if dist.is_available() and dist.is_initialized() else 1


def get_local_rank() -> int:
    return int(os.environ.get("LOCAL_RANK", "0"))


def print0(*a, **k):
    if get_rank() == 0:
        print(*a, **k)


def init_distributed_singlenode(timeout: int = 0, backend: str = None):
    world = int(os.environ.get("WORLD_SIZE", "1"))
    if world == 1 or "MASTER_ADDR" not in os.environ:
        return get_local_rank(), int(os.environ.get("RANK", "0")), 1
    rank, local = int(os.environ["RANK"]), get_local_rank()
    if backend is None:
        backend = "nccl" if torch.cuda.is_available() else "gloo"
    kw = {"timeout": timedelta(seconds=timeout)} if timeout else {}
    if backend == "nccl":
        torch.cuda.set_device(local)
    dist.init_process_group(backend=backend, init_method="env://", world_size=world, rank=rank, **kw)
    barrier(local)
    return local, rank, world


def barrier(local_rank: int = None):
    if dist.get_backend() == "nccl":
        dist.barrier(device_ids=[torch.cuda.current_device() if local_rank is None else local_rank])
    else:
        dist.barrier()


class GradReducer:

    def __init__(self, params, bucket_mb: float = 256.0, wire_dtype="auto", group=None, tail_mb: float = 8.0,
                 world_override: int = None, force_collectives: bool = False, head_mb: float = 64.0,
                 record_timeline: bool = False, late_params=None):
        self.params = [p for p in params if p.requires_grad]
        self.group = group
        self.nranks = dist.get_world_size(group) if dist.is_initialized() else 1
        if world_override is not None:
            self.nranks = int(world_override)
        self.world = self.nranks if not (force_collectives and self.nranks == 1 and dist.is_initialized()) else 2
        self._wire_auto = False
        if isinstance(wire_dtype, str):
            if wire_dtype != "auto":
                raise ValueError("wire_dtype: a torch dtype, None (fp32) or 'auto'")
            wire_dtype = None
        self.wire_dtype = wire_dtype
        self._wire = {}
        self._comm = None
        self._avg_ok = None
        self.record_timeline = bool(record_timeline)
        self._timeline = []
        self._t0 = None
        dev = self.params[0].device
        total = sum(p.numel() for p in self.params)
        self.flat = torch.zeros(total, dtype=torch.float32, device=dev)
        order = list(reversed(self.params))
        late = {id(p) for p in (late_params or [])}
        if late:
            order = [p for p in order if id(p) not in late] + [p for p in order if id(p) in late]
        self.order = order
        cap = max(1, int(bucket_mb * (1 << 20) / 4))
        tail = min(int(tail_mb * (1 << 20) / 4), cap)
        head = max(1, min(int(head_mb * (1 << 20) / 4), cap)) if head_mb else cap
        tail_from, acc = len(order), 0
        for i in range(len(order) - 1, -1, -1):
            acc += order[i].numel()
            if acc > tail:
                break
            tail_from = i
        self.buckets = []
        self._bucket_of = {}
        off = b_start = 0
        for i, p in enumerate(order):
            if i == tail_from and off > b_start:
                self.buckets.append((b_start, off))
                b_start = off
            n = p.numel()
            p.grad = self.flat[off:off + n].view_as(p)
            self._bucket_of[p] = len(self.buckets)
            off += n
            if off - b_start >= (head if not self.buckets else cap):
                self.buckets.append((b_start, off))
                b_start = off
        if off > b_start:
            self.buckets.append((b_start, off))
        self._slots = {p.data_ptr(): (p, p.grad) for p in self.params}
        self._grad_ptrs = [(p, p.grad.data_ptr()) for p in self.params]
        self._need = [0] * len(self.buckets)
        for p in order:
            self._need[self._bucket_of[p]] += 1
        self._pending = list(self._need)
        self._fired = {}
        self._deferred = set()
        self._streams = [set() for _ in self.buckets]
        self._work = []
        self._enabled = True
        if self.world > 1:
            for p in self.params:
                p.register_post_accumulate_grad_hook(self._hook)

    def slot(self, p):
        ent = self._slots.get(p.data_ptr())
        return ent[1] if ent is not None and ent[0].shape == p.shape else None

    def ready(self, p):
        if self.world > 1:
            self._count(self._slots[p.data_ptr()][0])

    def defer(self, p):
        if self.world > 1:
            self._deferred.add(id(self._slots[p.data_ptr()][0]))

    def rebind(self):
        self._slots = {p.data_ptr(): (p, p.grad) for p in self.params}

    def _hook(self, p):
        if id(p) in self._deferred:
            return
        self._count(p)

    def note_autocast(self, bf16: bool):
        return None

    def _comm_stream(self):
        if self._comm is None:
            self._comm = torch.cuda.Stream(device=self.flat.device)
        return self._comm

    def _post_stream(self):
        if getattr(self, "_post", None) is None:
            self._post = torch.cuda.Stream(device=self.flat.device)
        return self._post

    def _count(self, p):
        if not self._enabled:
            return
        b = self._bucket_of[p]
        if id(p) in self._fired:
            return
        self._fired[id(p)] = 1
        if p.is_cuda:
            self._streams[b].add(torch.cuda.current_stream())
        self._pending[b] -= 1
        if self._pending[b] == 0:
            self._launch(b)

    def _launch(self, b):
        s, e = self.buckets[b]
        buf = self.flat[s:e]
        if not buf.is_cuda:
            buf.div_(self.nranks)
            if self.wire_dtype is not None and self.wire_dtype != torch.float32:
                wire = buf.to(self.wire_dtype)
                h = dist.all_reduce(wire, op=dist.ReduceOp.SUM, group=self.group, async_op=True)
                self._work.append((h, buf, wire, None))
            else:
                h = dist.all_reduce(buf, op=dist.ReduceOp.SUM, group=self.group, async_op=True)
                self._work.append((h, None, None, None))
            return
        comm = self._comm_stream()
        for st in self._streams[b]:
            ev = torch.cuda.Event()
            ev.record(st)
            comm.wait_event(ev)
        self._streams[b] = set()
        post = self._post_stream()
        with torch.cuda.stream(comm):
            ev0 = None
            if self.record_timeline:
                if self._t0 is None:
                    self._t0 = torch.cuda.Event(enable_timing=True)
                    self._t0.record(comm)
                ev0 = torch.cuda.Event(enable_timing=True)
                ev0.record(comm)
            scale = 1.0 / self.nranks
            if self.wire_dtype is not None and self.wire_dtype != torch.float32:
                wire = self._wire.get(b)
                if wire is None:
                    wire = self._wire[b] = torch.empty(e - s, dtype=self.wire_dtype, device=buf.device)
                if self.nranks > 1:
                    torch.mul(buf, scale, out=wire)
                else:
                    wire.copy_(buf)
                h = dist.all_reduce(wire, op=dist.ReduceOp.SUM, group=self.group, async_op=True)
                nbytes = wire.numel() * wire.element_size()
            else:
                wire = None
                if self._avg_ok is None:
                    self._avg_ok = dist.get_backend(self.group) == "nccl" and hasattr(dist.ReduceOp, "AVG")
                if self._avg_ok and self.nranks > 1:
                    h = dist.all_reduce(buf, op=dist.ReduceOp.AVG, group=self.group, async_op=True)
                else:
                    if self.nranks > 1:
                        buf.mul_(scale)
                    h = dist.all_reduce(buf, op=dist.ReduceOp.SUM, group=self.group, async_op=True)
                nbytes = buf.numel() * 4
        with torch.cuda.stream(post):
            h.wait()
            if wire is not None:
                buf.copy_(wire)
            done = None
            if ev0 is not None:
                done = torch.cuda.Event(enable_timing=True)
                done.record(post)
                self._timeline.append([b, nbytes, ev0, done])
        self._work.append((h, None, None, ev0))

    def no_sync(self):
        reducer = self

        class _Ctx:
            def __enter__(self):
                reducer._enabled = False

            def __exit__(self, *a):
                reducer._enabled = True

        return _Ctx()

    def check_bound(self):
        for p, ptr in self._grad_ptrs:
            if p.grad is None or p.grad.data_ptr() != ptr:
                raise RuntimeError("a parameter's .grad no longer points into the GradReducer arena (zero_grad(set_to_none=True)?); "
                                   "use GradReducer.zero_grad()")

    def finish(self):
        self.check_bound()
        if self.world > 1 and self._enabled:
            if self._pending == self._need and not self._work:
                self._deferred = set()
                return
            missing = [b for b, n in enumerate(self._pending) if n != 0]
            if missing:
                lost = [(i, tuple(p.shape), self._fired.get(id(p), 0)) for i, p in enumerate(self.params) if self._fired.get(id(p), 0) != 1]
                raise RuntimeError("buckets %s did not receive all their gradients; parameters (index, shape) that "
                                   "did not report exactly once (index, shape, count): %s" % (missing, lost[:12]))
            if self._comm is not None and self.flat.is_cuda:
                torch.cuda.current_stream().wait_stream(self._post_stream())
            else:
                for h, buf, wire, _ in self._work:
                    h.wait()
                    if wire is not None:
                        buf.copy_(wire)
            self._work = []
            if self.record_timeline:
                self._last_timeline, self._last_t0 = self._timeline, self._t0
                self._timeline, self._t0 = [], None
            self._pending = list(self._need)
            self._fired = {}
        self._deferred = set()

    def mark(self, what):
        if self.record_timeline and self.flat.is_cuda and self.world > 1:
            ev = torch.cuda.Event(enable_timing=True)
            ev.record()
            setattr(self, "_" + what, ev)

    def backward_window_ms(self):
        b0, b1, t0 = getattr(self, "_bw0", None), getattr(self, "_bw1", None), getattr(self, "_last_t0", None)
        if b0 is None or b1 is None or t0 is None:
            return None
        torch.cuda.synchronize()
        return b0.elapsed_time(t0), b0.elapsed_time(b1)

    def timeline(self):
        tl, t0 = getattr(self, "_last_timeline", None), getattr(self, "_last_t0", None)
        if not tl or t0 is None:
            return []
        torch.cuda.synchronize()
        return [(b, nb, t0.elapsed_time(e0), t0.elapsed_time(e1) if e1 is not None else float("nan")) for b, nb, e0, e1 in tl]

    def zero_grad(self):
        self.flat.zero_()

    def broadcast_parameters(self, src: int = 0):
        if self.nranks == 1:
            return
        with torch.no_grad():
            chunk, acc = [], 0
            for p in self.params:
                chunk.append(p)
                acc += p.numel()
                if acc * 4 >= (256 << 20):
                    self._bcast(chunk, src)
                    chunk, acc = [], 0
            if chunk:
                self._bcast(chunk, src)

    def _bcast(self, ps, src):
        flat = torch.cat([p.detach().reshape(-1) for p in ps])
        dist.broadcast(flat, src, group=self.group)
        off = 0
        for p in ps:
            p.copy_(flat[off:off + p.numel()].view_as(p))
            off += p.numel()


class DataParallel(torch.nn.Module):

    _IGNORED = {"output_device", "dim", "broadcast_buffers", "process_group", "bucket_cap_mb", "check_reduction",
                "gradient_as_bucket_view", "init_sync", "device_mesh", "mixed_precision", "delay_all_reduce_named_params",
                "param_to_hook_all_reduce"}
    _UNSUPPORTED = {"find_unused_parameters", "static_graph"}

    def __init__(self, module, device_ids=None, bucket_mb: float = 256.0, wire_dtype="auto", tail_mb: float = 8.0,
                 force_collectives: bool = False, head_mb: float = 64.0, record_timeline: bool = False, **ddp_kwargs):
        super().__init__()
        for k, v in ddp_kwargs.items():
            if k in self._UNSUPPORTED:
                if v:
                    raise ValueError("mdm_hip.distributed.DataParallel does not implement %s=True: every parameter of the "
                                     "vision model must receive a gradient in every synchronised backward" % k)
            elif k not in self._IGNORED:
                raise TypeError("DataParallel got an unexpected keyword argument %r" % k)
        if ddp_kwargs.get("process_group") is not None:
            raise ValueError("process_group: pass the group to GradReducer directly (the default group is used here)")
        self.module = module
        net = getattr(module, "vision_model", module)
        late = net.late_gradient_parameters() if hasattr(net, "late_gradient_parameters") else None
        self.reducer = GradReducer(list(net.parameters()), bucket_mb=bucket_mb, wire_dtype=wire_dtype, tail_mb=tail_mb,
                                   force_collectives=force_collectives, head_mb=head_mb, record_timeline=record_timeline,
                                   late_params=late)
        self.reducer.broadcast_parameters(0)

    def forward(self, *args, **kwargs):
        return self.module(*args, **kwargs)

    def no_sync(self):
        return self.reducer.no_sync()
```

### ml-mdm_amd/mdm_hip/ops.py

```python
import ctypes
import weakref

import torch

from . import _lib
from . import tiling as _tiling

F32, BF16, F32_SPLIT, F32_SPLIT_W = 0, 1, 2, 3

_fp32_split = False
_weight_planes_on = True


class fp32_split:

    def __init__(self, enabled: bool = True):
        global _fp32_split
        self._prev = _fp32_split
        _fp32_split = bool(enabled)

    def __enter__(self):
        return self

    def __exit__(self, *a):
        global _fp32_split
        _fp32_split = self._prev


def fp32_split_enabled() -> bool:
    return _fp32_split


def _dt_mm(t: torch.Tensor) -> int:
    d = _dt(t)
    return F32_SPLIT if (d == F32 and _fp32_split) else d


def _dt(t: torch.Tensor) -> int:
    if t.dtype == torch.float32:
        return F32
    if t.dtype == torch.bfloat16:
        return BF16
    raise _lib.MdmHipError("unsupported activation dtype %s" % t.dtype)


def _epv(t: torch.Tensor) -> int:
    return 4 if t.dtype == torch.float32 else 8


def _p(t):
    return None if t is None else t.data_ptr()


_raw_stream = getattr(torch._C, "_cuda_getCurrentRawStream", None)
_raw_device = getattr(torch._C, "_cuda_getDevice", None)


def _stream():
    if _raw_stream is not None and _raw_device is not None:
        return _raw_stream(_raw_device())
    return torch.cuda.current_stream().cuda_stream


_stream_objs = {}


def _current_stream_obj():
    raw = _stream()
    st = _stream_objs.get(raw)
    if st is None:
        if len(_stream_objs) > 64:
            _stream_objs.clear()
        st = _stream_objs[raw] = torch.cuda.current_stream()
    return st


def _require_gpu(t: torch.Tensor):
    if not t.is_cuda:
        raise _lib.MdmHipError(
            "mdm_hip ops run only on an MI355X (got a %s tensor); there is no CPU fallback" % t.device
        )


def _f32_ws(nbytes: int, device):
    return torch.empty((max(int(nbytes), 4) + 3) // 4, dtype=torch.float32, device=device)


def _c(t):
    return t if t is None or t.is_contiguous() else t.contiguous()


_wcache = {}
_pack_epoch = 0


def invalidate_packed_weights():
    global _pack_epoch
    _pack_epoch += 1


_grad_sink = None


def set_grad_sink(sink):
    global _grad_sink
    if _grad_sink is not None and sink is not _grad_sink:
        flush_wgrad_queue()
    _grad_sink = sink


def _slot(param):
    if _grad_sink is None or param is None:
        return None
    return _grad_sink.slot(param)


def _sink_defer(param):
    f = getattr(_grad_sink, "defer", None)
    if f is not None and param is not None:
        f(param)


_side_stream = None
_async_wgrad = False


def enable_async_wgrad(flag: bool):
    global _async_wgrad
    _async_wgrad = bool(flag)


def side_stream():
    global _side_stream
    if _side_stream is None:
        _side_stream = torch.cuda.Stream()
    return _side_stream


_side_keep = []


def join_side_stream():
    if _side_stream is not None:
        torch.cuda.current_stream().wait_stream(_side_stream)
    _side_keep.clear()


def _off_critical_path(tensors, fn):
    if not (_async_wgrad and _grad_sink is not None):
        return fn()
    side = side_stream()
    if _raw_stream is None:
        side.wait_stream(torch.cuda.current_stream())
        with torch.cuda.stream(side):
            fn()
            done = torch.cuda.Event()
            done.record(side)
    else:
        cur = _current_stream_obj()
        side.wait_stream(cur)
        torch.cuda.set_stream(side)
        try:
            fn()
            done = torch.cuda.Event()
            done.record(side)
        finally:
            torch.cuda.set_stream(cur)
    live = [t for t in tensors if t is not None]
    _side_keep.append((done, live))
    if len(_side_keep) >= 64:
        _side_keep[:] = [e for e in _side_keep if not e[0].query()]


_defer_wgrad = False
_wgrad_queue = {}
_WG_MAX = 32


def enable_deferred_wgrad(flag: bool, max_group: int = 32):
    global _defer_wgrad, _WG_MAX
    flush_wgrad_queue()
    _defer_wgrad = bool(flag)
    _WG_MAX = max(1, min(32, int(max_group)))


def wgrad_grouped(xs, dys, dws, dbs=None):
    G = len(xs)
    M, cin = xs[0].shape
    cout = dys[0].shape[1]
    for t in list(xs) + list(dys):
        _require_gpu(t)
    xs, dys = [_c(t) for t in xs], [_c(t) for t in dys]
    arr = lambda vals: (ctypes.c_void_p * G)(*vals)
    _lib.check(_lib.lib().mdm_conv_wgrad_grouped(arr([_p(t) for t in xs]), arr([_p(t) for t in dys]), arr([_p(t) for t in dws]),
                                                 arr([_p(t) for t in dbs]) if dbs is not None else None, G, M, cin, cout,
                                                 _dt(xs[0]), _stream()), "mdm_conv_wgrad_grouped")


def _queue_wgrad(x, dy, weight, bias, slot, bslot, M, cin, cout):
    key = (M, cin, cout, x.device.index)
    q = _wgrad_queue.setdefault(key, [])
    q.append((x, dy, weight, bias, slot, bslot))
    _sink_defer(weight)
    if bslot is not None:
        _sink_defer(bias)
    if len(q) == _WG_MAX:
        _flush_key(key)


def _flush_key(key):
    q = _wgrad_queue.pop(key, None)
    if not q:
        return
    M, cin, cout, _ = key
    L = _lib.lib()
    tile = ctypes.c_int(0)
    _lib.check(L.mdm_conv_wgrad_group_plan(M, cout, cin, BF16, len(q), ctypes.byref(tile)), "mdm_conv_wgrad_group_plan")
    tensors = [t for e in q for t in (e[0], e[1])]
    if tile.value and all((e[5] is not None) == (q[0][5] is not None) for e in q):
        G = len(q)
        arr = lambda vals: (ctypes.c_void_p * G)(*vals)
        xs, dys, dws = arr([_p(e[0]) for e in q]), arr([_p(e[1]) for e in q]), arr([_p(e[4]) for e in q])
        dbs = arr([_p(e[5]) for e in q]) if q[0][5] is not None else None

        def go():
            _prof_wrap("conv_wgrad grouped x%d M=%d N=%d K=%d" % (G, M, cout, cin), 2.0 * G * M * cout * cin, lambda: _lib.check(
                L.mdm_conv_wgrad_grouped(xs, dys, dws, dbs, G, M, cin, cout, BF16, _stream()), "mdm_conv_wgrad_grouped"))
            for e in q:
                _grad_sink.ready(e[2])
                if e[5] is not None:
                    _grad_sink.ready(e[3])
    else:
        def go():
            for x, dy, w, b, slot, bslot in q:
                _wgrad_launch(x, dy, M, 1, 1, cin, 1, 1, cout, 1, 1, out=slot, dbias=bslot)
                _grad_sink.ready(w)
                if bslot is not None:
                    _grad_sink.ready(b)

    _off_critical_path(tensors, go)


def flush_wgrad_queue():
    for key in list(_wgrad_queue):
        _flush_key(key)
    flush_gn_params()


_gn_pending = []
_gn_pool = {}
_gn_tables = {}


def _gn_rows(N, C, device):
    ent = _gn_pool.get(device.index)
    need = 2 * N * C
    if ent is None or ent[1] + need > ent[0].numel():
        size = max(need, 0 if ent is None else 2 * ent[0].numel(), 16 << 20)
        ent = _gn_pool[device.index] = [torch.empty(size, dtype=torch.float32, device=device), 0]
    off = ent[1]
    ent[1] = off + need
    return ent[0][off:off + N * C], ent[0][off + N * C:off + need]


def flush_gn_params():
    if not _gn_pending:
        return
    dev = _gn_pending[0][0].device
    key = tuple((e[0].data_ptr(), e[1].data_ptr(), e[2].data_ptr(), e[3].data_ptr(), e[4], e[5]) for e in _gn_pending)
    ent = _gn_tables.get(key)
    if ent is None:
        import numpy as np
        rec = np.zeros(len(key), dtype=[("pg", "<u8"), ("pb", "<u8"), ("dg", "<u8"), ("db", "<u8"), ("N", "<i4"),
                                         ("C", "<i4"), ("first", "<i4"), ("pad", "<i4")])
        blocks = 0
        for i, (pg, pb, dg, db, N, C) in enumerate(key):
            rec[i] = (pg, pb, dg, db, N, C, blocks, 0)
            blocks += (C + 255) // 256
        table = torch.from_numpy(rec.view(np.uint8).copy()).to(dev)
        if len(_gn_tables) > 64:
            _gn_tables.clear()
        ent = _gn_tables[key] = (table, blocks)
    table, blocks = ent
    _lib.check(_lib.lib().mdm_gn_param_reduce_multi(_p(table), len(key), blocks, _stream()), "mdm_gn_param_reduce_multi")
    for e in _gn_pending:
        _grad_sink.ready(e[6])
        _grad_sink.ready(e[7])
    _gn_pending.clear()
    for ent in _gn_pool.values():
        ent[1] = 0


class _FlushPointFn(torch.autograd.Function):

    @staticmethod
    def forward(ctx, x):
        return x.view_as(x)

    @staticmethod
    def backward(ctx, dy):
        flush_wgrad_queue()
        return dy


def wgrad_flush_point(x):
    return _FlushPointFn.apply(x) if (_defer_wgrad and x.requires_grad) else x


def _wgrad_into_sink(x, dy, weight, bias, slot, bslot, N, H, W, cin, Ho, Wo, cout, ks, stride):
    M = N * Ho * Wo
    if _defer_wgrad and _async_wgrad and ks == 1 and x.dtype == torch.bfloat16 and M >= 4096:
        _queue_wgrad(x.reshape(M, cin), dy.reshape(M, cout), weight, bias, slot, bslot, M, cin, cout)
        return

    def go():
        _wgrad_launch(x, dy, N, H, W, cin, Ho, Wo, cout, ks, stride, out=slot, dbias=bslot)
        _grad_sink.ready(weight)
        if bslot is not None:
            _grad_sink.ready(bias)

    _off_critical_path((x, dy), go)


def _cache_slot(weight):
    k = id(weight)
    ent = _wcache.get(k)
    if ent is None or ent[0]() is not weight:
        ent = (weakref.ref(weight, lambda _r, k=k: _wcache.pop(k, None)), {})
        _wcache[k] = ent
    return ent[1]


def _round_up(v, m):
    return (v + m - 1) // m * m


def packed_weight(weight: torch.Tensor, bias, dtype: torch.dtype, forward_only: bool = False):
    key = (dtype, "fwd") if forward_only else dtype
    ent = _cache_slot(weight)
    ver = (weight._version, None if bias is None else bias._version, weight.data_ptr(), _pack_epoch)
    if key in ent and ent[key][0] == ver:
        return ent[key][1]
    _require_gpu(weight)
    L = _lib.lib()
    cout, cin = weight.shape[0], weight.shape[1]
    ks = weight.shape[2] if weight.dim() == 4 else 1
    epv = 4 if dtype == torch.float32 else 8
    cin_pad, cout_pad = _round_up(cin, epv), _round_up(cout, epv)
    taps = ks * ks
    w32 = _c(weight.detach().float())
    need_d = cin_pad == cin and not forward_only
    prev = ent[key][1] if key in ent else None
    if prev is not None and prev[0].numel() == cout_pad * taps * cin_pad and prev[0].device == weight.device:
        wf, wd = prev[0], prev[1]
    else:
        wf = torch.empty(cout_pad * taps * cin_pad, dtype=dtype, device=weight.device)
        wd = torch.empty(cin * taps * cout_pad, dtype=dtype, device=weight.device) if need_d else None
        if cout_pad != cout:
            wf.zero_()
    bk = 32 if dtype == torch.float32 else 64
    kbf = bk if (ks == 3 and cin_pad % bk == 0) else 0
    kbd = bk if (ks == 3 and cout_pad % bk == 0) else 0
    _lib.check(
        L.mdm_pack_weight(_p(w32), _p(wf), _p(wd), cout, cin, ks, cin_pad, cout_pad, kbf, kbd,
                          F32 if dtype == torch.float32 else BF16, _stream()),
        "mdm_pack_weight",
    )
    _repacked(wf, wd)
    bp = None
    if bias is not None:
        bp = bias.detach().float()
        if cout_pad != cout:
            bp = torch.cat([bp, bp.new_zeros(cout_pad - cout)])
        bp = _c(bp)
    val = (wf, wd, bp, cin_pad, cout_pad, kbf, kbd)
    ent[key] = (ver, val)
    return val


def packed_s2_dgrad_weight(weight: torch.Tensor):
    ent = _cache_slot(weight)
    ver = (weight._version, weight.data_ptr(), _pack_epoch)
    if "s2dgrad" in ent and ent["s2dgrad"][0] == ver:
        return ent["s2dgrad"][1]
    cout, cin = weight.shape[0], weight.shape[1]
    w = weight.detach()
    if w.dtype != torch.float32 or not w.is_contiguous():
        w = w.float().contiguous()
    old = ent.get("s2dgrad")
    packed = old[1] if old is not None and old[1].shape == (4 * cin, cout // 64, 4, 64) else \
        torch.empty((4 * cin, cout // 64, 4, 64), dtype=torch.bfloat16, device=w.device)
    _lib.check(_lib.lib().mdm_s2dgrad_pack(_p(w), _p(packed), cout, cin, _stream()), "mdm_s2dgrad_pack")
    ent["s2dgrad"] = (ver, packed)
    return packed


_multi_tables = {}


def repack_all(dtype: torch.dtype):
    import numpy as np

    items = []
    for wref, ent in _wcache.values():
        w = wref()
        if w is None or dtype not in ent or not w.is_cuda:
            continue
        ver, val = ent[dtype]
        wf, wd, bp, cin_pad, cout_pad, kbf, kbd = val
        cout, cin = w.shape[0], w.shape[1]
        if cin_pad != cin or cout_pad != cout or cin % 32 or cout % 32 or w.dtype != torch.float32 or not w.is_contiguous():
            continue
        taps = w.shape[2] * w.shape[3] if w.dim() == 4 else 1
        if taps not in (1, 9):
            continue
        items.append((w, ent, ver, val, cout, cin, taps, kbf, kbd))
    if not items:
        return
    sig = tuple((w.data_ptr(), val[0].data_ptr(), 0 if val[1] is None else val[1].data_ptr()) for w, _, _, val, *_ in items)
    tab = _multi_tables.get(dtype)
    if tab is None or tab[0] != sig:
        desc = np.zeros(len(items), dtype=[("w", "u8"), ("wf", "u8"), ("wd", "u8"), ("cout", "i4"), ("cin", "i4"),
                                           ("taps", "i4"), ("kbf", "i4"), ("kbd", "i4"), ("first", "i4")])
        first = 0
        for i, (w, _, _, val, cout, cin, taps, kbf, kbd) in enumerate(items):
            desc[i] = (w.data_ptr(), val[0].data_ptr(), 0 if val[1] is None else val[1].data_ptr(), cout, cin, taps, kbf, kbd, first)
            first += (cout // 32) * (cin // 32)
        assert desc.dtype.itemsize == 48
        dev_tab = torch.from_numpy(desc.view(np.uint8).copy()).to(items[0][0].device)
        tab = (sig, dev_tab, len(items), first)
        _multi_tables[dtype] = tab
    _lib.check(_lib.lib().mdm_pack_weights_multi(_p(tab[1]), tab[2], tab[3], F32 if dtype == torch.float32 else BF16, _stream()),
               "mdm_pack_weights_multi")
    for w, ent, ver, val, *_ in items:
        ent[dtype] = ((w._version, ver[1], w.data_ptr(), _pack_epoch), val)
        _repacked(val[0], val[1])


_prof = None
_prof_shapes = False


def profile_begin(shapes: bool = False):
    global _prof, _prof_shapes
    _prof, _prof_shapes = [], shapes


def _prof_wrap(name, work, fn, kind="mfma", executed=None):
    if _prof is None:
        return fn()
    e0, e1 = torch.cuda.Event(enable_timing=True), torch.cuda.Event(enable_timing=True)
    e0.record()
    r = fn()
    e1.record()
    if kind == "mfma":
        real = _lib.lib().mdm_last_gemm_kernel()
        if real:
            name = real.decode() + (name[name.index(" M="):] if " M=" in name else "")
    _prof.append((kind, name, work, e0, e1, work if executed is None else executed))
    return r


def profile_end(peak_tflops, peak_gbs=8000.0):
    global _prof
    rec, _prof = _prof, None
    torch.cuda.synchronize()
    agg, hbm = {}, {}
    for kind, name, work, e0, e1, executed in rec:
        a = (hbm if kind == "hbm" else agg).setdefault(name, [0, 0.0, 0.0, 0.0])
        a[0] += 1
        a[1] += work
        a[2] += e0.elapsed_time(e1) * 1e-3
        a[3] += executed
    if not agg:
        return None
    table = {k: {"launches": v[0], "alg_tflop": round(v[1] / 1e12, 3), "time_ms": round(v[2] * 1e3, 3),
                 "tflops": round(v[1] / v[2] / 1e12, 1)} for k, v in agg.items()}
    for k, v in agg.items():
        if abs(v[3] - v[1]) > 1e-6 * v[1]:
            table[k]["executed_tflops"] = round(v[3] / v[2] / 1e12, 1)
            table[k]["tflops_is"] = "credit for the dense 3x3 layer this sub-pixel kernel replaces (%.2fx the FLOPs it executes)" % (v[1] / v[3])
    dom = max(agg, key=lambda k: agg[k][2])
    n, fl, t = agg[dom][:3]
    ach = fl / t / 1e12
    tot_f, tot_t = sum(v[1] for v in agg.values()), sum(v[2] for v in agg.values())
    return {
        "bound": "mfma", "achieved": round(ach, 1), "peak": peak_tflops, "unit": "TFLOP/s", "frac": round(ach / peak_tflops, 4),
        "traffic": None, "kernel": dom, "dominant_by": "largest total time among the GEMM-class kernels of one step",
        "launches_per_step": n, "avg_launch_ms": round(t / n * 1e3, 4),
        "alg_gflop_per_launch": round(fl / n / 1e9, 2),
        "gemm_weighted": {"alg_tflop": round(tot_f / 1e12, 2), "time_ms": round(tot_t * 1e3, 2),
                          "tflops": round(tot_f / tot_t / 1e12, 1), "frac": round(tot_f / tot_t / 1e12 / peak_tflops, 4)},
        "all_gemm_kernels": table,
        "hbm_kernels": {k: {"launches": v[0], "alg_gb": round(v[1] / 1e9, 3), "time_ms": round(v[2] * 1e3, 3),
                            "gb_per_s": round(v[1] / v[2] / 1e9, 1), "frac_of_peak": round(v[1] / v[2] / 1e9 / peak_gbs, 4)}
                        for k, v in hbm.items()},
    }


_conv_plans = {}


def _conv_plan(M, Cout, K, dt):
    key = (M, Cout, K, dt)
    ent = _conv_plans.get(key)
    if ent is None:
        sp, wsb = ctypes.c_int(1), ctypes.c_size_t(0)
        _lib.check(_lib.lib().mdm_conv_fwd_plan(M, Cout, K, dt, ctypes.byref(sp), ctypes.byref(wsb)), "mdm_conv_fwd_plan")
        ent = _conv_plans[key] = (sp.value, wsb.value)
    return ent


def _repacked(*packs):
    for t in packs:
        if t is not None:
            t._mdm_serial = getattr(t, "_mdm_serial", 0) + 1


def _weight_planes(w: torch.Tensor):
    ent, serial = getattr(w, "_mdm_planes", None), getattr(w, "_mdm_serial", 0)
    if ent is not None and ent[0] == serial:
        return ent[1]
    planes = torch.empty_like(w)
    _lib.check(_lib.lib().mdm_split_weight_planes(_p(w), _p(planes), w.numel(), _stream()), "mdm_split_weight_planes")
    w._mdm_planes = (serial, planes)
    return planes


def _conv_launch(x, w, bias, res, aux, y, ypre, N, H, W, Cin, Ho, Wo, Cout, ks, stride, transposed, act, kblk=0):
    splits, wsb = _conv_plan(N * Ho * Wo, Cout, ks * ks * Cin, _dt(x)) if (stride == 1 and not transposed) else (1, 0)
    ws = _f32_ws(wsb, x.device) if splits > 1 else None
    dt = _dt_mm(x)
    if dt == F32_SPLIT and (ks * ks * Cin) % 8 == 0 and w.numel() % 8 == 0 and _weight_planes_on:
        w, dt = _weight_planes(w), F32_SPLIT_W

    def go():
        _lib.check(
            _lib.lib().mdm_conv_fwd_ws(_p(x), _p(w), _p(bias), _p(res), _p(aux), _p(y), _p(ypre), N, H, W, Cin, Ho, Wo, Cout,
                                       ks, stride, transposed, act, kblk, dt, _p(ws), wsb, _stream()),
            "mdm_conv_fwd",
        )

    if _prof is None:
        return go()
    code = _lib.lib().mdm_conv_fwd_tile(N * Ho * Wo, Cout, _dt(x))
    mode = "1x1" if ks == 1 else ("3x3_T2" if transposed else "3x3")
    name = "conv_gemm_kernel<%s,%dx%d,%s>" % ("f32" if x.dtype == torch.float32 else "bf16", code // 1000, code % 1000, mode)
    flops = 2.0 * N * Ho * Wo * Cout * ks * ks * Cin / (4 if transposed else 1)
    if _prof_shapes:
        name += " M=%d N=%d K=%d" % (N * Ho * Wo, Cout, ks * ks * Cin)
    return _prof_wrap(name, flops, go)


def _wgrad_launch(x, dy, N, H, W, Cin, Ho, Wo, Cout, ks, stride, out=None, dbias=None):
    L = _lib.lib()
    splits = ctypes.c_int(0)
    wsb = ctypes.c_size_t(0)
    M, K = N * Ho * Wo, ks * ks * Cin
    _lib.check(L.mdm_conv_wgrad_plan(M, Cout, K, _dt(x), ctypes.byref(splits), ctypes.byref(wsb)), "mdm_conv_wgrad_plan")
    ws = _f32_ws(wsb.value, x.device)
    dw = torch.empty((Cout, Cin, ks, ks), dtype=torch.float32, device=x.device) if out is None else out

    def go():
        _lib.check(L.mdm_conv_wgrad(_p(x), _p(dy), 0 if dbias is None else 1, _p(ws), N, H, W, Cin, Ho, Wo, Cout, ks, stride,
                                    _dt(x), _stream()),
                   "mdm_conv_wgrad")

    if _prof is None:
        go()
    else:
        te = L.mdm_conv_wgrad_tile(M, Cout, K, _dt(x))
        kn = "conv_wgrad_kernel" if x.dtype == torch.float32 else "conv_wgrad_tr_kernel"
        name = "%s<%s,%dx%d,%s>" % (kn, "f32" if x.dtype == torch.float32 else "bf16", te, te, "1x1" if ks == 1 else "3x3")
        if _prof_shapes:
            name += " M=%d N=%d K=%d" % (M, Cout, K)
        _prof_wrap(name, 2.0 * M * Cout * K, go)
    _lib.check(L.mdm_conv_wgrad_reduce(_p(ws), _p(dw), _p(dbias), _p(dy), M, Cin, Cout, ks, 0 if out is None else 1, _dt(x),
                                       _stream()), "mdm_conv_wgrad_reduce")
    return dw


def _colsum_launch(x2d, M, C, out=None):
    L = _lib.lib()
    nb = ctypes.c_int(0)
    wsb = ctypes.c_size_t(0)
    _lib.check(L.mdm_colsum_plan(M, C, ctypes.byref(nb), ctypes.byref(wsb)), "mdm_colsum_plan")
    ws = _f32_ws(wsb.value, x2d.device)
    acc = 0 if out is None else 1
    if out is None:
        out = torch.empty(C, dtype=torch.float32, device=x2d.device)
    _lib.check(L.mdm_colsum(_p(x2d), _p(out), _p(ws), M, C, acc, _dt(x2d), _stream()), "mdm_colsum")
    return out


def _geom(x, ks, stride):
    if x.dim() == 2:
        return x.shape[0], 1, 1, 1, 1
    N, H, W = x.shape[0], x.shape[1], x.shape[2]
    if ks == 1:
        return N, H, W, H, W
    return N, H, W, (H - 1) // stride + 1, (W - 1) // stride + 1


def _out_shape(x, Ho, Wo, C):
    return (x.shape[0], C) if x.dim() == 2 else (x.shape[0], Ho, Wo, C)


def _conv_forward(x, weight, bias, residual, stride):
    ks = weight.shape[2] if weight.dim() == 4 else 1
    wf, wd, bp, cin_pad, cout_pad, kbf, kbd = packed_weight(weight, bias, x.dtype)
    if x.shape[-1] != cin_pad:
        raise _lib.MdmHipError("conv input has %d channels, packed weight expects %d" % (x.shape[-1], cin_pad))
    N, H, W, Ho, Wo = _geom(x, ks, stride)
    y = torch.empty(_out_shape(x, Ho, Wo, cout_pad), dtype=x.dtype, device=x.device)
    _conv_launch(x, wf, bp, residual, None, y, None, N, H, W, cin_pad, Ho, Wo, cout_pad, ks, stride, 0, 0, kbf)
    return y, ks


class ConvFn(torch.autograd.Function):

    @staticmethod
    def forward(ctx, x, weight, bias, residual, stride, tap=False):
        _require_gpu(x)
        x = _c(x)
        residual = _c(residual)
        y, ks = _conv_forward(x, weight, bias, residual, stride)
        ctx.save_for_backward(x, weight, bias)
        ctx.stride, ctx.ks = stride, ks
        ctx.has_res = residual is not None
        if tap:
            ctx.set_materialize_grads(False)
            return y, x.view_as(x)
        return y

    @staticmethod
    def backward(ctx, dy, dtap=None):
        x, weight, bias = ctx.saved_tensors
        if dy is None:
            raise _lib.MdmHipError("conv(tap=True): the convolution's own output received no gradient")
        return _conv_backward(ctx, x, weight, bias, dy, dtap) + (None, None)


def _conv_backward(ctx, x, weight, bias, dy, dtap=None):
    dy = _c(dy)
    dtap = _c(dtap)
    ks, stride = ctx.ks, ctx.stride
    wf, wd, bp, cin_pad, cout_pad, kbf, kbd = packed_weight(weight, bias, x.dtype)
    cout, cin = weight.shape[0], weight.shape[1]
    N, H, W, Ho, Wo = _geom(x, ks, stride)
    dx = dw = db = None
    if ctx.needs_input_grad[0]:
        if wd is None:
            raise _lib.MdmHipError("input gradient requested for a channel-padded convolution")
        dx = torch.empty_like(x)
        if ks == 3 and stride == 2 and x.dtype == torch.bfloat16 and cout_pad == cout and cout % 64 == 0 and cin % 128 == 0 \
                and H % 2 == 0 and W % 2 == 0:
            wsel = packed_s2_dgrad_weight(weight)
            _prof_wrap("conv_gemm_bl_kernel<sel4> (3x3 stride-2 input gradient) M=%d N=%d K=%d" % (N * Ho * Wo, 4 * cin, 4 * cout),
                       2.0 * N * Ho * Wo * cout * 9 * cin, lambda: _lib.check(
                _lib.lib().mdm_conv_s2_dgrad_res(_p(dy), _p(wsel), _p(dtap), _p(dx), N, Ho, Wo, cout, cin, BF16, _stream()),
                "mdm_conv_s2_dgrad_res"), executed=2.0 * N * Ho * Wo * (4 * cin) * (4 * cout))
            dtap = None
        elif ks == 3 and stride == 2:
            _conv_launch(dy, wd, None, None, None, dx, None, N, Ho, Wo, cout_pad, H, W, cin, 3, 1, 1, 0, kbd)
        else:
            _conv_launch(dy, wd, None, None, None, dx, None, N, Ho, Wo, cout_pad, H, W, cin, ks, 1, 0, 0, kbd)
        if dtap is not None:
            dx = dx + dtap
    elif dtap is not None:
        dx = dtap
    padded = cout_pad != cout or cin_pad != cin
    want_b = bias is not None and ctx.needs_input_grad[2]
    if ctx.needs_input_grad[1]:
        slot = None if padded else _slot(weight)
        bslot = _slot(bias) if (slot is not None and want_b) else None
        if slot is not None:
            _wgrad_into_sink(x, dy, weight, bias, slot, bslot, N, H, W, cin_pad, Ho, Wo, cout_pad, ks, stride)
            if bslot is not None:
                want_b = False
        else:
            dbt = torch.empty(cout_pad, dtype=torch.float32, device=x.device) if want_b else None
            dwp = _wgrad_launch(x, dy, N, H, W, cin_pad, Ho, Wo, cout_pad, ks, stride, dbias=dbt)
            if padded:
                dwp = dwp[:cout, :cin].contiguous()
            dw = dwp.view(weight.shape)
            if want_b:
                db = dbt[:cout]
                want_b = False
    if want_b:
        slot = None if cout_pad != cout else _slot(bias)
        if slot is not None:
            _colsum_launch(dy, N * Ho * Wo, cout_pad, out=slot)
            _grad_sink.ready(bias)
        else:
            db = _colsum_launch(dy, N * Ho * Wo, cout_pad)[:cout]
    dres = dy if (ctx.has_res and ctx.needs_input_grad[3]) else None
    return dx, dw, db, dres


def conv(x, weight, bias=None, residual=None, stride=1):
    return ConvFn.apply(x, weight, bias, residual, stride)


def conv_tap(x, weight, bias=None, stride=1):
    if not (torch.is_grad_enabled() and x.requires_grad):
        return ConvFn.apply(x, weight, bias, None, stride), x
    return ConvFn.apply(x, weight, bias, None, stride, True)


STEM_DGRAD_MAX_CIN = 8


def conv3x3_stem_dgrad(dy, weight, bias=None):
    _require_gpu(dy)
    dy = _c(dy)
    if weight.dim() != 4 or weight.shape[2] != 3 or weight.shape[3] != 3:
        raise _lib.MdmHipError("conv3x3_stem_dgrad: a 3x3 convolution weight is expected")
    cin = weight.shape[1]
    if not 1 <= cin <= STEM_DGRAD_MAX_CIN:
        raise _lib.MdmHipError("input gradient of a channel-padded stem convolution is implemented for at most %d input "
                               "channels (got %d)" % (STEM_DGRAD_MAX_CIN, cin))
    wf, _, _, cin_pad, cout_pad, kbf, _ = packed_weight(weight, bias, dy.dtype)
    if dy.dim() != 4 or dy.shape[-1] != cout_pad or kbf:
        raise _lib.MdmHipError("conv3x3_stem_dgrad: dy %s does not match the packed weight (%d channels)"
                               % (tuple(dy.shape), cout_pad))
    N, H, W = dy.shape[0], dy.shape[1], dy.shape[2]
    dx = torch.empty((N, cin, H, W), dtype=torch.float32, device=dy.device)

    def go():
        _lib.check(_lib.lib().mdm_conv3x3_stem_dgrad(_p(dy), _p(wf), _p(dx), N, H, W, cout_pad, cin, _dt(dy), _stream()),
                   "mdm_conv3x3_stem_dgrad")

    if _prof is None:
        go()
    else:
        name = "stem_dgrad_kernel<%s,%d>" % ("f32" if dy.dtype == torch.float32 else "bf16", cin)
        if _prof_shapes:
            name += " M=%d N=%d K=%d" % (N * H * W, cin, 9 * cout_pad)
        _prof_wrap(name, float(dy.numel() * dy.element_size() + dx.numel() * 4), go, kind="hbm")
    return dx


class StemConvFn(torch.autograd.Function):

    @staticmethod
    def forward(ctx, x, weight, bias, dtype):
        _require_gpu(x)
        x = _c(x.float())
        N, C, H, W = x.shape
        epv = 4 if dtype == torch.float32 else 8
        xh = torch.empty((N, H, W, _round_up(C, epv)), dtype=dtype, device=x.device)
        _lib.check(_lib.lib().mdm_nchw_to_nhwc(_p(x), _p(xh), N, C, H, W, xh.shape[-1], _dt(xh), _stream()), "mdm_nchw_to_nhwc")
        y, _ = _conv_forward(xh, weight, bias, None, 1)
        ctx.save_for_backward(xh, weight, bias)
        return y

    @staticmethod
    def backward(ctx, dy):
        xh, weight, bias = ctx.saved_tensors
        nig = ctx.needs_input_grad
        dy = _c(dy)
        dx = conv3x3_stem_dgrad(dy, weight, bias) if nig[0] else None
        _, dw, db, _ = _conv_backward(_ConvNeeds(3, 1, False, (False, nig[1], nig[2], False)), xh, weight, bias, dy)
        return dx, dw, db, None


def stem_conv(x_nchw, weight, bias=None, dtype=torch.float32):
    if weight.dim() != 4 or weight.shape[2] != 3:
        raise _lib.MdmHipError("stem_conv: a 3x3 convolution weight is expected")
    cin = weight.shape[1]
    if x_nchw.dim() != 4 or x_nchw.shape[1] != cin:
        raise _lib.MdmHipError("stem_conv: input %s vs weight %s" % (tuple(x_nchw.shape), tuple(weight.shape)))
    if cin > STEM_DGRAD_MAX_CIN:
        if cin % (4 if dtype == torch.float32 else 8) == 0:
            return conv(to_nhwc(x_nchw, dtype), weight, bias)
        raise _lib.MdmHipError("input gradient of a channel-padded stem convolution is implemented for at most %d input "
                               "channels (got %d)" % (STEM_DGRAD_MAX_CIN, cin))
    return StemConvFn.apply(x_nchw, weight, bias, dtype)


def packed_upconv_weights(weight: torch.Tensor, bias):
    ent = _cache_slot(weight)
    ver = (weight._version, None if bias is None else bias._version, weight.data_ptr(), _pack_epoch)
    if "upconv" in ent and ent["upconv"][0] == ver:
        return ent["upconv"][1]
    cout, cin = weight.shape[0], weight.shape[1]
    prev = ent["upconv"][1] if "upconv" in ent else None
    if prev is not None and prev[0].device == weight.device:
        w_ph, w_t = prev[0], prev[1]
    else:
        w_ph = torch.empty(4 * cout * 4 * cin, dtype=torch.bfloat16, device=weight.device)
        w_t = torch.empty(cin * 16 * cout, dtype=torch.bfloat16, device=weight.device)
    _lib.check(_lib.lib().mdm_upconv_pack(_p(_c(weight.detach().float())), _p(w_ph), _p(w_t), cout, cin, _stream()), "mdm_upconv_pack")
    bias4 = _c(bias.detach().float().repeat(4)) if bias is not None else None
    val = (w_ph, w_t, bias4)
    ent["upconv"] = (ver, val)
    return val


def upsample_conv_supported(x, weight):
    return x.is_cuda and x.dtype == torch.bfloat16 and x.dim() == 4 and weight.dim() == 4 and weight.shape[2] == 3 and \
        weight.shape[0] % 256 == 0 and weight.shape[1] % 256 == 0 and x.shape[-1] == weight.shape[1] and \
        (x.shape[1] & (x.shape[1] - 1)) == 0 and (x.shape[2] & (x.shape[2] - 1)) == 0


class UpsampleConvFn(torch.autograd.Function):

    @staticmethod
    def forward(ctx, x, weight, bias):
        _require_gpu(x)
        x = _c(x)
        N, H, W, cin = x.shape
        cout = weight.shape[0]
        w_ph, _, bias4 = packed_upconv_weights(weight, bias)
        y = torch.empty((N, 2 * H, 2 * W, cout), dtype=x.dtype, device=x.device)
        _prof_wrap("conv_gemm_bl_kernel<sel4> (upsample2x + 3x3) M=%d N=%d K=%d" % (N * H * W, 4 * cout, 4 * cin),
                   2.0 * N * 4 * H * W * cout * 9 * cin, lambda: _lib.check(
            _lib.lib().mdm_conv_up_fwd(_p(x), _p(w_ph), _p(bias4), _p(y), N, H, W, cin, cout, BF16, _stream()), "mdm_conv_up_fwd"),
                   executed=2.0 * N * H * W * (4 * cout) * (4 * cin))
        ctx.save_for_backward(x, weight, bias)
        return y

    @staticmethod
    def backward(ctx, dy):
        x, weight, bias = ctx.saved_tensors
        dy = _c(dy)
        N, H, W, cin = x.shape
        cout = weight.shape[0]
        L = _lib.lib()
        _, w_t, _ = packed_upconv_weights(weight, bias)
        dyb = torch.empty((N, H, W, 4 * cout), dtype=dy.dtype, device=dy.device)
        _lib.check(L.mdm_space_to_depth2x(_p(dy), _p(dyb), N, H, W, cout, BF16, _stream()), "mdm_space_to_depth2x")
        dx = dw = db = None
        if ctx.needs_input_grad[0]:
            dx = torch.empty_like(x)
            _prof_wrap("conv_gemm_bl_kernel<sel4> (upsample2x + 3x3 input gradient) M=%d N=%d K=%d" % (N * H * W, cin, 16 * cout),
                       2.0 * N * 4 * H * W * cout * 9 * cin, lambda: _lib.check(
                L.mdm_conv_up_dgrad(_p(dyb), _p(w_t), _p(dx), N, H, W, cout, cin, BF16, _stream()), "mdm_conv_up_dgrad"),
                           executed=2.0 * N * H * W * cin * (16 * cout))
        if ctx.needs_input_grad[1]:
            want_b = bias is not None and ctx.needs_input_grad[2]
            slot = _slot(weight)
            bslot = _slot(bias) if (slot is not None and want_b) else None
            sunk = slot is not None and (bslot is not None or not want_b)
            M, K = N * H * W, 9 * cin
            splits, wsb = ctypes.c_int(0), ctypes.c_size_t(0)
            _lib.check(L.mdm_conv_wgrad_plan(M, 4 * cout, K, BF16, ctypes.byref(splits), ctypes.byref(wsb)), "mdm_conv_wgrad_plan")

            def go():
                ws = _f32_ws(wsb.value, x.device)
                dwb = torch.empty((4 * cout, cin, 3, 3), dtype=torch.float32, device=x.device)
                db4 = torch.empty(4 * cout, dtype=torch.float32, device=x.device) if want_b else None
                _prof_wrap("conv_wgrad_bl_kernel<1, 1> (upsample2x + 3x3, 16 of 36 blocks) M=%d N=%d K=%d" % (M, 4 * cout, K),
                           2.0 * 4 * M * cout * K, lambda: _lib.check(
                    L.mdm_conv_wgrad_blocked(_p(x), _p(dyb), 1 if want_b else 0, _p(ws), N, H, W, cin, cout, BF16, _stream()),
                    "mdm_conv_wgrad_blocked"), executed=2.0 * 4 * M * cout * K * 16.0 / 36.0)
                _lib.check(L.mdm_conv_wgrad_reduce(_p(ws), _p(dwb), _p(db4), _p(dyb), M, cin, 4 * cout, 3, 0, BF16, _stream()),
                           "mdm_conv_wgrad_reduce")
                dwo = slot if sunk else torch.empty(weight.shape, dtype=torch.float32, device=x.device)
                dbo = (bslot if sunk else torch.empty(cout, dtype=torch.float32, device=x.device)) if want_b else None
                _lib.check(L.mdm_upconv_wfold(_p(dwb), _p(dwo), _p(db4), _p(dbo), cout, cin, 1 if sunk else 0, _stream()), "mdm_upconv_wfold")
                if sunk:
                    _grad_sink.ready(weight)
                    if want_b:
                        _grad_sink.ready(bias)
                return dwo, dbo

            if sunk:
                _off_critical_path((x, dyb), go)
            else:
                dw, db = go()
        return dx, dw, db


def upsample_conv(x, weight, bias=None):
    if upsample_conv_supported(x, weight):
        return UpsampleConvFn.apply(x, weight, bias)
    return ConvFn.apply(upsample2x(x), weight, bias, None, 1)


def linear(x, weight, bias=None, residual=None):
# ... 1896 lines not shown
```

### ml-mdm_amd/mdm_hip/trainer.py

```python
import collections
import math
import os

import torch

from . import ops
from .distributed import DataParallel, GradReducer


class FusedState:

    def __init__(self, net, reducer=None, bucket_mb=256.0, wire_dtype="auto", use_ema=True, async_wgrad=True):
        self.net = net
        self.params = [p for p in net.parameters() if p.requires_grad]
        late = net.late_gradient_parameters() if hasattr(net, "late_gradient_parameters") else None
        self.reducer = reducer if reducer is not None else GradReducer(self.params, bucket_mb=bucket_mb, wire_dtype=wire_dtype,
                                                                       late_params=late)
        self.reducer.broadcast_parameters(0)
        flat = torch.empty_like(self.reducer.flat)
        self.slices = {}
        off = 0
        with torch.no_grad():
            for p in self.reducer.order:
                n = p.numel()
                flat[off:off + n].copy_(p.reshape(-1))
                p.data = flat[off:off + n].view_as(p)
                self.slices[id(p)] = (off, n)
                off += n
        self.flat_p = flat
        self.m = torch.zeros_like(flat)
        self.v = torch.zeros_like(flat)
        self.flat_ema = flat.clone() if use_ema else None
        self.gnorm_sq = torch.zeros(1, dtype=torch.float32, device=flat.device)
        self.step_dev = torch.zeros(1, dtype=torch.int32, device=flat.device)
        self.reducer.rebind()
        self.async_wgrad = async_wgrad
        self._host_vals = {}
        self.activate()

    def activate(self):
        ops.set_grad_sink(self.reducer)
        ops.enable_async_wgrad(self.async_wgrad)
        ops.enable_deferred_wgrad(self.async_wgrad, max_group=32 if self.reducer.world == 1 else 13)
        ops.invalidate_packed_weights()

    def view(self, arena, p):
        off, n = self.slices[id(p)]
        return arena[off:off + n].view_as(p)

    def finish_backward(self):
        ops.flush_wgrad_queue()
        self.reducer.mark("bw1")
        ops.join_side_stream()
        self.reducer.finish()

    def post_scalar(self, name, value):
        ent = self._host_vals.get(name)
        if ent is None:
            ent = (torch.empty(1, dtype=torch.float32).pin_memory(), torch.cuda.Event())
            self._host_vals[name] = ent
        ent[0].copy_(value.detach().reshape(1), non_blocking=True)
        ent[1].record()

    def read_scalar(self, name):
        buf, ev = self._host_vals[name]
        ev.synchronize()
        return float(buf[0])

    def post_skip_flag(self):
        ring = self.__dict__.setdefault("_skip_ring", [])
        k = self.__dict__.get("_skip_next", 0)
        if len(ring) <= k:
            ring.append((torch.empty(1, dtype=torch.float32).pin_memory(), torch.cuda.Event()))
        buf, ev = ring[k]
        self._skip_next = (k + 1) % 4
        buf.copy_(self.gnorm_sq.detach().reshape(1), non_blocking=True)
        ev.record()
        return buf, ev

    def optimizer_step(self, lr, betas, eps, weight_decay, clip_norm, ema_decay, dtype, loss=None):
        if loss is not None and self.reducer.world == 1:
            self.reducer.flat[:1].add_(loss.detach().float().reshape(1) * 0.0)
        ops.sumsq(self.reducer.flat, out=self.gnorm_sq, step_counter=self.step_dev)
        ops.adamw_ema_step(self.flat_p, self.reducer.flat, self.m, self.v, self.flat_ema, self.gnorm_sq, lr, betas[0], betas[1],
                           eps, weight_decay, 0, clip_norm, ema_decay, zero_grad=True, step_dev=self.step_dev)
        ops.repack_all(dtype)


def _vision_model(model):
    core = getattr(model.model, "module", model.model)
    return core.vision_model


def _adopt(model, optimizer, ema_model):
    st = getattr(optimizer, "_mdm_fused", None)
    if st is not None:
        if st is not False and st.ema_id != (id(ema_model) if ema_model is not None else None):
            raise RuntimeError("train_batch was first called %s and now %s: pass the same ema_model on every call "
                               "(the fused step adopted it together with the optimizer)"
                               % ("without an ema_model" if st.ema_id is None else "with another ema_model",
                                  "without one" if ema_model is None else "with one"))
        return st if st is not False else None

    def no(reason):
        optimizer._mdm_fused = False
        optimizer._mdm_fused_reason = reason
        return None

    from .unet import UNet

    wrapped = model.model
    net = _vision_model(model)
    if isinstance(wrapped, torch.nn.parallel.DistributedDataParallel):
        return no("torch DistributedDataParallel owns the gradient buckets (use mdm_hip.distributed.DataParallel)")
    if not isinstance(net, UNet):
        return no("vision model is not an mdm_hip UNet")
    params = [p for p in net.parameters() if p.requires_grad]
    if not params:
        return no("vision model has no trainable parameters")
    if not all(p.is_cuda and p.dtype == torch.float32 for p in params):
        return no("parameters are not fp32 tensors on the GPU")
    if type(optimizer) not in (torch.optim.AdamW, torch.optim.Adam) or len(optimizer.param_groups) != 1:
        return no("optimizer is not a single-group torch Adam / AdamW")
    grp = optimizer.param_groups[0]
    if grp.get("amsgrad") or grp.get("maximize") or (type(optimizer) is torch.optim.Adam and grp.get("weight_decay", 0) != 0
                                                      and not grp.get("decoupled_weight_decay", False)):
        return no("optimizer options without a fused counterpart (amsgrad / maximize / L2 weight decay)")
    if [id(p) for p in grp["params"]] != [id(p) for p in params]:
        return no("optimizer does not hold exactly the vision model's parameters")
    ema_net = None
    if ema_model is not None:
        ema_net = ema_model.module
        if getattr(ema_model, "device", None) is not None or set(net.state_dict()) != {n for n, _ in net.named_parameters()} or \
                [(n, tuple(p.shape)) for n, p in ema_net.named_parameters()] != [(n, tuple(p.shape)) for n, p in net.named_parameters()]:
            return no("ModelEma on another device / of another shape / with persistent buffers")
    reducer = wrapped.reducer if isinstance(wrapped, DataParallel) else \
        GradReducer(params, group=None, world_override=1)
    if [id(p) for p in reducer.params] != [id(p) for p in params]:
        return no("the DataParallel wrapper's reducer does not hold exactly the vision model's parameters")
    had_state = {id(p): dict(optimizer.state.get(p, {})) for p in params}
    st = FusedState(net, reducer=reducer, use_ema=ema_net is not None, async_wgrad=os.environ.get("MDM_HIP_SERIAL_WGRAD", "0") != "1")
    with torch.no_grad():
        steps = 0
        for p in params:
            old = had_state[id(p)]
            mv, vv = st.view(st.m, p), st.view(st.v, p)
            if "exp_avg" in old:
                mv.copy_(old["exp_avg"])
                vv.copy_(old["exp_avg_sq"])
                steps = max(steps, int(old["step"]))
            optimizer.state[p] = {"step": None, "exp_avg": mv, "exp_avg_sq": vv}
        st.step_dev.fill_(steps)
        step_host = torch.tensor(float(steps))
        for p in params:
            optimizer.state[p]["step"] = step_host
        optimizer.register_state_dict_pre_hook(lambda opt, st=st, t=step_host: (_settle(st, keep=0), t.fill_(float(int(st.step_dev)))) and None)

        def _reinstall(opt, st=st, params=params, t=step_host):
            with torch.no_grad():
                steps_ = 0
                for p_ in params:
                    ent = opt.state.get(p_)
                    if not ent or "exp_avg" not in ent:
                        continue
                    mv_, vv_ = st.view(st.m, p_), st.view(st.v, p_)
                    if ent["exp_avg"].data_ptr() != mv_.data_ptr():
                        mv_.copy_(ent["exp_avg"])
                        vv_.copy_(ent["exp_avg_sq"])
                    steps_ = max(steps_, int(ent["step"]))
                    opt.state[p_] = {"step": t, "exp_avg": mv_, "exp_avg_sq": vv_}
                st.step_dev.fill_(steps_)
                t.fill_(float(steps_))

        optimizer.register_load_state_dict_post_hook(_reinstall)
        if ema_net is not None:
            by_name = dict(net.named_parameters())
            for name, pe in ema_net.named_parameters():
                ev = st.view(st.flat_ema, by_name[name])
                ev.copy_(pe.detach())
                pe.data = ev
    st.ema_id = id(ema_model) if ema_model is not None else None
    optimizer._mdm_fused = st
    return st


def _loss_of(losses, weights):
    return losses.mean() if weights is None else (losses * weights).sum() / weights.sum()


def _clip_parameters(model, optimizer):
    mine = list(model.model.parameters())
    seen = {id(p) for p in mine}
    extra = []
    for grp in optimizer.param_groups:
        for p in grp["params"]:
            if id(p) not in seen:
                seen.add(id(p))
                extra.append(p)
    return mine + extra if extra else model.model.parameters()


def train_batch(model, sample, optimizer, scheduler, logger, args, grad_scaler=None, accumulate_gradient=False,
                num_grad_accumulations=1, ema_model=None, loss_factor=1.0):
    model.train()
    lr = scheduler.get_last_lr()[0]
    st = _adopt(model, optimizer, ema_model)
    if st is None and isinstance(model.model, DataParallel):
        raise RuntimeError("mdm_hip.distributed.DataParallel only works with the fused train step, which this call cannot "
                           "take: %s.  Use torch.optim.AdamW / Adam (one parameter group, no amsgrad) with a ModelEma on "
                           "the model's device, or wrap the model in torch.nn.parallel.DistributedDataParallel instead."
                           % getattr(optimizer, "_mdm_fused_reason", "?"))
    fp16 = bool(getattr(args, "fp16", False))
    dev_type = "cuda" if next(_vision_model(model).parameters()).is_cuda else "cpu"
    if st is not None:
        return _train_batch_fused(st, model, sample, optimizer, scheduler, logger, args, accumulate_gradient,
                                  num_grad_accumulations, ema_model, loss_factor, lr, fp16)
    if fp16:
        with torch.autocast(dev_type, dtype=torch.bfloat16):
            losses, times, x_t, means, targets, weights = model.get_loss(sample)
            loss = _loss_of(losses, weights) * loss_factor
            loss_val = loss.item()
            if math.isnan(loss_val):
                optimizer.zero_grad()
                return loss_val, losses, times, x_t, means, targets
            if num_grad_accumulations != 1:
                loss = loss / num_grad_accumulations
        if grad_scaler is not None:
            grad_scaler.scale(loss).backward()
        else:
            loss.backward()
    else:
        losses, times, x_t, means, targets, weights = model.get_loss(sample)
        loss = _loss_of(losses, weights)
        loss_val = loss.item()
        if math.isnan(loss_val):
            optimizer.zero_grad()
            optimizer.step()
            scheduler.step()
            return loss_val, losses, times, x_t, means, targets
        loss.backward()

    if not accumulate_gradient:
        clip = float(getattr(args, "gradient_clip_norm", 2.0))
        core = getattr(model.model, "module", model.model)
        if fp16 and grad_scaler is not None:
            grad_scaler.unscale_(optimizer)
            optimizer._mdm_grad_norm = torch.nn.utils.clip_grad_norm_(_clip_parameters(model, optimizer), clip)
            grad_scaler.step(optimizer)
            grad_scaler.update()
        else:
            optimizer._mdm_grad_norm = torch.nn.utils.clip_grad_norm_(_clip_parameters(model, optimizer), clip)
            optimizer.step()
        ops.invalidate_packed_weights()
        if ema_model is not None:
            ema_model.update(core.vision_model)
        if logger is not None:
            logger.add_scalar("train/Loss", loss_val)
            logger.add_scalar("lr", lr)
        optimizer.zero_grad()
        scheduler.step()
    return loss_val, losses, times, x_t, means, targets


def _train_batch_fused(st, model, sample, optimizer, scheduler, logger, args, accumulate_gradient, num_grad_accumulations,
                       ema_model, loss_factor, lr, fp16):
    lockstep = st.reducer.world > 1 and not accumulate_gradient
    _settle(st)
    if ops._grad_sink is not st.reducer:
        st.activate()
    st.reducer.note_autocast(fp16)
    with torch.autocast("cuda", dtype=torch.bfloat16, enabled=fp16):
        losses, times, x_t, means, targets, weights = model.get_loss(sample)
        loss = _loss_of(losses, weights)
        if fp16:
            loss = loss * loss_factor
        st.post_scalar("loss", loss)
        if fp16 and num_grad_accumulations != 1:
            loss = loss / num_grad_accumulations
    st.reducer.mark("bw0")
    loss.backward()
    st.finish_backward()
    if not accumulate_gradient:
        grp = optimizer.param_groups[0]
        decay = 0.0
        if ema_model is not None:
            decay = float(ema_model.counter >= ema_model.warmup_steps) * ema_model.decay
        st.optimizer_step(grp["lr"], grp["betas"], grp["eps"], grp["weight_decay"], float(getattr(args, "gradient_clip_norm", 2.0)),
                          decay, torch.bfloat16 if fp16 else torch.float32, loss=loss)
        optimizer._opt_called = True
        skip_flag = st.post_skip_flag()
    loss_val = st.read_scalar("loss")
    if not lockstep and math.isnan(loss_val):
        return _fused_nan_return(st, optimizer, scheduler, fp16, loss_val, losses, times, x_t, means, targets, accumulate_gradient)
    if not accumulate_gradient:
        if ema_model is not None:
            ema_model.counter += 1
        if logger is not None:
            logger.add_scalar("train/Loss", loss_val)
            logger.add_scalar("lr", lr)
        scheduler.step()
    if not accumulate_gradient:
        st.__dict__.setdefault("unsettled", collections.deque()).append((skip_flag, scheduler, ema_model, fp16))
        if _STRICT_NAN:
            _settle(st, keep=0)
    return loss_val, losses, times, x_t, means, targets


_STRICT_NAN = os.environ.get("MDM_HIP_STRICT_NAN", "0") == "1"


def _settle(st, keep=1):
    pend = getattr(st, "unsettled", None)
    while pend is not None and len(pend) > keep:
        (buf, ev), scheduler, ema_model, fp16 = pend.popleft()
        ev.synchronize()
        if math.isfinite(float(buf[0])):
            continue
        if ema_model is not None:
            ema_model.counter -= 1
        if fp16:
            closed = getattr(scheduler, "_get_closed_form_lr", None)
            scheduler.last_epoch -= 1
            if hasattr(scheduler, "_step_count"):
                scheduler._step_count -= 1
            lrs = closed() if closed is not None else scheduler.get_lr()
            for g, lr in zip(scheduler.optimizer.param_groups, lrs):
                g["lr"] = lr
            scheduler._last_lr = [g["lr"] for g in scheduler.optimizer.param_groups]


def _fused_nan_return(st, optimizer, scheduler, fp16, loss_val, losses, times, x_t, means, targets, clear):
    if clear:
        _skip_step(st, optimizer, None, False, None, fp16)
    if not fp16:
        scheduler.step()
    return loss_val, losses, times, x_t, means, targets



def _skip_step(st, optimizer, loss, accumulate_gradient, args, fp16):
    st.finish_backward()
    st.reducer.zero_grad()


class ModelEma(torch.nn.Module):

    def __init__(self, model, decay=0.9999, warmup_steps=0, device=None):
        super().__init__()
        from copy import deepcopy

        self.module = deepcopy(model)
        self.module.eval()
        self.decay, self.device, self.warmup_steps, self.counter = decay, device, warmup_steps, 0
        if device is not None:
            self.module.to(device=device)

    def update(self, model):
        decay = (self.counter >= self.warmup_steps) * self.decay
        self.counter += 1
        with torch.no_grad():
            msd = model.state_dict()
            for k, ema_v in self.module.state_dict().items():
                mv = msd[k].detach()
                if self.device:
                    mv = mv.to(device=self.device)
                ema_v.mul_(decay).add_(mv, alpha=1.0 - decay)

    def save(self, fname, other_items=None):
        ckpt = {"state_dict": self.module.state_dict()}
        ckpt.update(other_items or {})
        torch.save(ckpt, fname)

    def load(self, fname):
        ckpt = torch.load(fname, map_location="cpu")
        mine = self.module.state_dict()
        self.module.load_state_dict({k: v for k, v in ckpt["state_dict"].items() if k in mine}, strict=False)


class TrainStep:

    def __init__(self, pipeline, lr=5e-5, clip_norm=2.0, ema_decay=0.9999, bf16=True, use_ema=True,
                 bucket_mb=256.0, wire_dtype=None, fused=None, betas=(0.9, 0.999), eps=1e-8, weight_decay=0.0,
                 async_wgrad=True):
        self.pipeline = pipeline
        self.net = pipeline.get_model().vision_model
        self.params = [p for p in self.net.parameters() if p.requires_grad]
        self.fused = self.params[0].is_cuda if fused is None else fused
        self.lr, self.betas, self.eps, self.weight_decay = lr, betas, eps, weight_decay
        self.clip_norm, self.bf16, self.ema_decay = clip_norm, bf16, ema_decay
        self.steps = 0
        if self.fused:
            pipeline.materialize_targets = False
            self.state = FusedState(self.net, bucket_mb=bucket_mb, wire_dtype=wire_dtype, use_ema=use_ema, async_wgrad=async_wgrad)
            self.reducer = self.state.reducer
            self.opt = None
            self.ema = None
        else:
            self.reducer = GradReducer(self.params, bucket_mb=bucket_mb, wire_dtype=wire_dtype)
            self.reducer.broadcast_parameters(0)
            self.opt = torch.optim.AdamW(self.params, lr=lr, betas=betas, weight_decay=weight_decay, eps=eps)
            self.ema = [p.detach().clone() for p in self.params] if use_ema else None

    flat_p = property(lambda self: self.state.flat_p)
    m = property(lambda self: self.state.m)
    v = property(lambda self: self.state.v)
    flat_ema = property(lambda self: self.state.flat_ema)
    step_dev = property(lambda self: self.state.step_dev)

    def ema_state(self):
        names = {id(p): n for n, p in self.net.named_parameters()}
        if self.fused:
            return {names[id(p)]: self.state.view(self.state.flat_ema, p) for p in self.params}
        return {names[id(p)]: e for p, e in zip(self.params, self.ema)}

    def __call__(self, sample, **loss_kw):
        self.pipeline.train()
        dev_type = "cuda" if self.params[0].is_cuda else "cpu"
        with torch.autocast(dev_type, dtype=torch.bfloat16, enabled=self.bf16):
            losses, times, x_t, means, targets, weights = self.pipeline.get_loss(sample, **loss_kw)
            loss = _loss_of(losses, weights)
        if self.fused:
            self.state.reducer.note_autocast(self.bf16)
            self.state.post_scalar("loss", loss)
            loss.backward()
            self.state.finish_backward()
            self.state.optimizer_step(self.lr, self.betas, self.eps, self.weight_decay, self.clip_norm, self.ema_decay,
                                      torch.bfloat16 if self.bf16 else torch.float32, loss=loss)
            loss_val = self.state.read_scalar("loss")
            self.steps += 1 if math.isfinite(loss_val) else 0
            return loss_val
        loss_val = loss.item()
        bad = not math.isfinite(loss_val)
        if self.reducer.world > 1:
            flag = torch.tensor([1.0 if bad else 0.0], device=self.params[0].device)
            torch.distributed.all_reduce(flag, op=torch.distributed.ReduceOp.MAX, group=self.reducer.group)
            bad = bool(flag.item() > 0)
        if bad:
            self.reducer.zero_grad()
            return loss_val
        loss.backward()
        ops.flush_wgrad_queue()
        ops.join_side_stream()
        self.reducer.finish()
        self.steps += 1
        gnorm = torch.linalg.vector_norm(self.reducer.flat)
        scale = torch.clamp(self.clip_norm / (gnorm + 1e-6), max=1.0)
        self.reducer.flat.mul_(scale)
        self.opt.step()
        ops.invalidate_packed_weights()
        if self.ema is not None:
            with torch.no_grad():
                torch._foreach_lerp_(self.ema, [p.detach() for p in self.params], 1.0 - self.ema_decay)
        self.reducer.zero_grad()
        return loss_val
```

Baseline: 11.45 steps/s.

## Store ResNet 3x3 conv weights tap-major and group their weight-gradient kernels

ResNet conv1/conv2 weights and gradients now live in the parameter arena in a tap-major (O, kh, kw, I) layout. This lets the 3x3 weight-gradient GEMM write directly in its natural K order, so deferred 3x3 wgrads can be batched into one grouped launch. Weight packing and split-K reduction gain tap-major source and destination variants, including a wider 8-way unrolled reduce kernel. The cost is extra layout bookkeeping in the optimizer, EMA and state_dict paths, strided parameter views, and an env opt-out back to OIHW.

```diff
diff --git a/include/mdm_hip_ext.h b/include/mdm_hip_ext.h
--- a/include/mdm_hip_ext.h
+++ b/include/mdm_hip_ext.h
@@ -52,6 +52,13 @@
                         float* h1, float* psum, float* x0_out, float* x_last_out, int B, size_t chw, int pred_type, int clip,
                         float image_scale, int max_predictor, int max_corrector, void* stream);
 
+int mdm_conv_wgrad_reduce_tm(const float* ws, float* dw_tm, float* dbias, const void* dy, int M, int Cin, int Cout,
+                             int ksize, int accumulate, int dtype, void* stream);
+int mdm_pack_weight_tm(const float* w_tm, void* w_fwd, void* w_dgrad, int Cout, int Cin, int ksize, int Cin_pad,
+                       int Cout_pad, int kblock_fwd, int kblock_dgrad, int dtype, void* stream);
+int mdm_conv_wgrad_grouped3x3(const void* const* x, const void* const* dy, float* const* dw_tm, float* const* dbias,
+                              int groups, int N, int H, int W, int Cin, int Cout, int dtype, void* stream);
+
 #ifdef __cplusplus
 }
 #endif
diff --git a/ml-mdm_amd/csrc/gemm_conv.hip b/ml-mdm_amd/csrc/gemm_conv.hip
--- a/ml-mdm_amd/csrc/gemm_conv.hip
+++ b/ml-mdm_amd/csrc/gemm_conv.hip
@@ -1491,9 +1491,36 @@
   }
 }
 
+__global__ __launch_bounds__(192) void wgrad_reduce_tm_kernel(const float* __restrict__ slab, float* __restrict__ dw,
+                                                              const float* __restrict__ bslab, float* __restrict__ dbias,
+                                                              int splits, int Cout, size_t total, int accumulate,
+                                                              int wblocks, int bblocks) {
+  if ((int)blockIdx.x < bblocks) {
+    __shared__ float part[192];
+    wgrad_bias_reduce<192>(bslab, dbias, splits, Cout, accumulate, (int)blockIdx.x, part);
+    return;
+  }
+  const size_t n4 = total / 4;
+  const f32x4* s4 = reinterpret_cast<const f32x4*>(slab);
+  f32x4* d4 = reinterpret_cast<f32x4*>(dw);
+  for (size_t i = (size_t)(blockIdx.x - bblocks) * 192 + threadIdx.x; i < n4; i += (size_t)wblocks * 192) {
+    f32x4 acc[8];
+#pragma unroll
+    for (int u = 0; u < 8; ++u) acc[u] = f32x4{0.f, 0.f, 0.f, 0.f};
+    int sp = 0;
+    for (; sp + 8 <= splits; sp += 8) {
+#pragma unroll
+      for (int u = 0; u < 8; ++u) acc[u] += s4[(size_t)(sp + u) * n4 + i];
+    }
+    for (; sp < splits; ++sp) acc[0] += s4[(size_t)sp * n4 + i];
+    const f32x4 a = ((acc[0] + acc[1]) + (acc[2] + acc[3])) + ((acc[4] + acc[5]) + (acc[6] + acc[7]));
+    d4[i] = accumulate ? d4[i] + a : a;
+  }
+}
+
 template <typename T>
 __global__ void pack_weight_kernel(const float* __restrict__ w, T* __restrict__ wf, T* __restrict__ wd,
-                                   int Cout, int Cin, int taps, int Cin_pad, int Cout_pad, int kbf, int kbd) {
+                                   int Cout, int Cin, int taps, int Cin_pad, int Cout_pad, int kbf, int kbd, int src_tm) {
   const size_t Kf = (size_t)taps * Cin_pad, Kd = (size_t)taps * Cout_pad;
   const size_t total_f = (size_t)Cout * Kf;
   const size_t total_d = wd ? (size_t)Cin * Kd : 0;
@@ -1505,7 +1532,7 @@
       int tp, i;
       if (kbf) { const int cb = kpos / (taps * kbf), r = kpos - cb * taps * kbf; tp = r / kbf; i = cb * kbf + (r - tp * kbf); }
       else { tp = kpos / Cin_pad; i = kpos - tp * Cin_pad; }
-      wf[idx] = from_f32<T>(i < Cin ? w[((size_t)o * Cin + i) * taps + tp] : 0.f);
+      wf[idx] = from_f32<T>(i < Cin ? (src_tm ? w[((size_t)o * taps + tp) * Cin + i] : w[((size_t)o * Cin + i) * taps + tp]) : 0.f);
     } else {
       const size_t d = idx - total_f;
       const int i = (int)(d / Kd);
@@ -1513,7 +1540,7 @@
       int tp, o;
       if (kbd) { const int ob = kpos / (taps * kbd), r = kpos - ob * taps * kbd; tp = r / kbd; o = ob * kbd + (r - tp * kbd); }
       else { tp = kpos / Cout_pad; o = kpos - tp * Cout_pad; }
-      wd[d] = from_f32<T>(o < Cout ? w[((size_t)o * Cin + i) * taps + (taps - 1 - tp)] : 0.f);
+      wd[d] = from_f32<T>(o < Cout ? (src_tm ? w[((size_t)o * taps + (taps - 1 - tp)) * Cin + i] : w[((size_t)o * Cin + i) * taps + (taps - 1 - tp)]) : 0.f);
     }
   }
 }
@@ -1521,13 +1548,21 @@
 template <typename T, int TAPS>
 __global__ __launch_bounds__(256) void pack_weight_tiled_kernel(const float* __restrict__ w, T* __restrict__ wf,
                                                                 T* __restrict__ wd, int Cout, int Cin, int kbf,
-                                                                int kbd) {
+                                                                int kbd, int src_tm) {
   __shared__ float tile[32][32 * TAPS + 1];
   const int ib = blockIdx.x * 32, ob = blockIdx.y * 32;
   const int tid = threadIdx.x;
-  for (int e = tid; e < 32 * 32 * TAPS; e += 256) {
-    const int ol = e / (32 * TAPS), r = e - ol * (32 * TAPS);
-    tile[ol][r] = w[((size_t)(ob + ol) * Cin + ib) * TAPS + r];
+  if (src_tm) {
+    for (int e = tid; e < 32 * 32 * TAPS; e += 256) {
+      const int ol = e / (32 * TAPS), r = e - ol * (32 * TAPS);
+      const int tp = r >> 5, il = r & 31;
+      tile[ol][il * TAPS + tp] = w[((size_t)(ob + ol) * TAPS + tp) * Cin + ib + il];
+    }
+  } else {
+    for (int e = tid; e < 32 * 32 * TAPS; e += 256) {
+      const int ol = e / (32 * TAPS), r = e - ol * (32 * TAPS);
+      tile[ol][r] = w[((size_t)(ob + ol) * Cin + ib) * TAPS + r];
+    }
   }
   __syncthreads();
   const size_t Kf = (size_t)TAPS * Cin, Kd = (size_t)TAPS * Cout;
@@ -1556,6 +1591,7 @@
   int Cout, Cin, taps, kbf, kbd;
   int first_block;
 };
+constexpr int PACK_SRC_TM = 0x100;
 
 template <typename T, int TAPS>
 __device__ __forceinline__ void pack_brick(const PackDesc& d, int brick, float (*tile)[32 * 9 + 1]) {
@@ -1564,11 +1600,21 @@
   const int ib = (brick % ibn) * 32, ob = (brick / ibn) * 32;
   const int tid = threadIdx.x;
   const int Cin = d.Cin, Cout = d.Cout;
-  for (int e = tid; e < 32 * 8 * TAPS; e += 256) {
-    const int ol = e / (8 * TAPS), q = e - ol * (8 * TAPS);
-    const f32x4 v = *reinterpret_cast<const f32x4*>(d.w + ((size_t)(ob + ol) * Cin + ib) * TAPS + q * 4);
-#pragma unroll
-    for (int j = 0; j < 4; ++j) tile[ol][q * 4 + j] = v[j];
+  if (d.taps & PACK_SRC_TM) {
+    for (int e = tid; e < 32 * 8 * TAPS; e += 256) {
+      const int ol = e / (8 * TAPS), q = e - ol * (8 * TAPS);
+      const int tp = q >> 3, i4 = (q & 7) * 4;
+      const f32x4 v = *reinterpret_cast<const f32x4*>(d.w + ((size_t)(ob + ol) * TAPS + tp) * Cin + ib + i4);
+#pragma unroll
+      for (int j = 0; j < 4; ++j) tile[ol][(i4 + j) * TAPS + tp] = v[j];
+    }
+  } else {
+    for (int e = tid; e < 32 * 8 * TAPS; e += 256) {
+      const int ol = e / (8 * TAPS), q = e - ol * (8 * TAPS);
+      const f32x4 v = *reinterpret_cast<const f32x4*>(d.w + ((size_t)(ob + ol) * Cin + ib) * TAPS + q * 4);
+#pragma unroll
+      for (int j = 0; j < 4; ++j) tile[ol][q * 4 + j] = v[j];
+    }
   }
   __syncthreads();
   const size_t Kf = (size_t)TAPS * Cin, Kd = (size_t)TAPS * Cout;
@@ -1608,7 +1654,7 @@
     if (table[mid].first_block <= b) lo = mid; else hi = mid - 1;
   }
   const PackDesc d = table[lo];
-  if (d.taps == 9) pack_brick<T, 9>(d, b - d.first_block, tile);
+  if ((d.taps & ~PACK_SRC_TM) == 9) pack_brick<T, 9>(d, b - d.first_block, tile);
   else pack_brick<T, 1>(d, b - d.first_block, tile);
 }
 
@@ -2632,40 +2678,62 @@
   return 0;
 }
 
-extern "C" int mdm_conv_wgrad_grouped(const void* const* x, const void* const* dy, float* const* dw,
-                                      float* const* dbias, int groups, int M, int Cin, int Cout, int dtype,
-                                      void* stream) {
+static int wgrad_grouped_impl(const void* const* x, const void* const* dy, float* const* dw, float* const* dbias,
+                              int groups, int N, int H, int W, int Cin, int Cout, int ksize, int dtype, void* stream) {
   MDM_CHECK_ARG(x && dy && dw && groups >= 1 && groups <= WG_MAXG);
-  MDM_CHECK_ARG(dtype == DT_BF16 && Cin % 8 == 0 && Cout % 8 == 0 && M > 0);
+  MDM_CHECK_ARG(dtype == DT_BF16 && Cin % 8 == 0 && Cout % 8 == 0 && N > 0 && H > 0 && W > 0);
+  MDM_CHECK_ARG((size_t)N * H * W <= 0x7FFFFFFFu);
+  const int M = N * H * W, K = ksize * ksize * Cin;
   WgradArgs a = {};
-  a.N = M; a.H = 1; a.W = 1; a.Cin = Cin; a.Ho = 1; a.Wo = 1; a.Cout = Cout; a.stride = 1;
-  a.M = M; a.K = Cin; a.splits = 1; a.groups = groups;
+  a.N = N; a.H = H; a.W = W; a.Cin = Cin; a.Ho = H; a.Wo = W; a.Cout = Cout; a.stride = 1;
+  a.M = M; a.K = K; a.splits = 1; a.groups = groups;
   a.mtiles_per_split = (M + 63) / 64;
-  MDM_CHECK_ARG(wgrad_bl_ok(a, 1));
+  MDM_CHECK_ARG(wgrad_bl_ok(a, ksize));
   WgradGroup gr = {};
   for (int g = 0; g < groups; ++g) {
     MDM_CHECK_ARG(x[g] && dy[g] && dw[g]);
     gr.x[g] = x[g]; gr.dy[g] = dy[g]; gr.out[g] = dw[g]; gr.bout[g] = dbias ? dbias[g] : nullptr;
   }
-  int te = wgrad_group_tile(M, Cout, Cin, groups);
-  if (!te) te = wgrad_forced_tile(Cout, Cin, DT_BF16);
-  if (!te) te = (Cout >= 192 && Cin >= 192) ? 256 : 128;
-  const int tiles = ((Cout + te - 1) / te) * ((Cin + te - 1) / te);
+  int te = wgrad_group_tile(M, Cout, K, groups);
+  if (!te) te = wgrad_forced_tile(Cout, K, DT_BF16);
+  if (!te) te = (Cout >= 192 && K >= 192) ? 256 : 128;
+  const int tiles = ((Cout + te - 1) / te) * ((K + te - 1) / te);
   hipStream_t st = reinterpret_cast<hipStream_t>(stream);
   constexpr int smem = 4 * 128 * 128, smem_big = 4 * 64 * 512;
+  const int mode = ksize == 1 ? MODE_1x1 : MODE_3x3;
   if (te == 256) {
-    ensure_dynamic_lds(conv_wgrad_bl_kernel<MODE_1x1, 1>, smem_big);
-    hipLaunchKernelGGL((conv_wgrad_bl_kernel<MODE_1x1, 1>), dim3(tiles * groups), dim3(512), smem_big, st, a, gr);
-  } else {
+    if (ksize == 1) {
+      ensure_dynamic_lds(conv_wgrad_bl_kernel<MODE_1x1, 1>, smem_big);
+      hipLaunchKernelGGL((conv_wgrad_bl_kernel<MODE_1x1, 1>), dim3(tiles * groups), dim3(512), smem_big, st, a, gr);
+    } else {
+      ensure_dynamic_lds(conv_wgrad_bl_kernel<MODE_3x3, 1>, smem_big);
+      hipLaunchKernelGGL((conv_wgrad_bl_kernel<MODE_3x3, 1>), dim3(tiles * groups), dim3(512), smem_big, st, a, gr);
+    }
+  } else if (ksize == 1) {
     ensure_dynamic_lds(conv_wgrad_bl_kernel<MODE_1x1, 0>, smem);
     hipLaunchKernelGGL((conv_wgrad_bl_kernel<MODE_1x1, 0>), dim3(tiles * groups), dim3(256), smem, st, a, gr);
-  }
-  MDM_NOTE_KERNEL("conv_wgrad_bl_kernel<%d, %d>", MODE_1x1, te == 256 ? 1 : 0);
+  } else {
+    ensure_dynamic_lds(conv_wgrad_bl_kernel<MODE_3x3, 0>, smem);
+    hipLaunchKernelGGL((conv_wgrad_bl_kernel<MODE_3x3, 0>), dim3(tiles * groups), dim3(256), smem, st, a, gr);
+  }
+  MDM_NOTE_KERNEL("conv_wgrad_bl_kernel<%d, %d>", mode, te == 256 ? 1 : 0);
   MDM_LAUNCH_STATUS();
 }
 
-extern "C" int mdm_conv_wgrad_reduce(const float* ws, float* dw_oihw, float* dbias, const void* dy, int M, int Cin,
-                                     int Cout, int ksize, int accumulate, int dtype, void* stream) {
+extern "C" int mdm_conv_wgrad_grouped(const void* const* x, const void* const* dy, float* const* dw,
+                                      float* const* dbias, int groups, int M, int Cin, int Cout, int dtype,
+                                      void* stream) {
+  return wgrad_grouped_impl(x, dy, dw, dbias, groups, M, 1, 1, Cin, Cout, 1, dtype, stream);
+}
+
+extern "C" int mdm_conv_wgrad_grouped3x3(const void* const* x, const void* const* dy, float* const* dw_tm,
+                                         float* const* dbias, int groups, int N, int H, int W, int Cin, int Cout,
+                                         int dtype, void* stream) {
+  return wgrad_grouped_impl(x, dy, dw_tm, dbias, groups, N, H, W, Cin, Cout, 3, dtype, stream);
+}
+
+static int wgrad_reduce_impl(const float* ws, float* dw_oihw, float* dbias, const void* dy, int M, int Cin,
+                             int Cout, int ksize, int accumulate, int dtype, int dst_tm, void* stream) {
   MDM_CHECK_ARG(ws && dw_oihw && (ksize == 1 || ksize == 3));
   const int K = ksize * ksize * Cin;
   int splits; size_t wsb;
@@ -2680,6 +2748,12 @@
     const int wblocks = (int)((total / 4 + 255) / 256 > 2048 ? 2048 : (total / 4 + 255) / 256);
     hipLaunchKernelGGL(wgrad_reduce_flat_kernel, dim3(wblocks + bblocks), dim3(256), 0, st, ws, dw_oihw, bslab, dbias,
                        splits, Cout, total, accumulate, wblocks, bblocks);
+  } else if (dst_tm) {
+    MDM_CHECK_ARG(Cin % 4 == 0);
+    const size_t total = (size_t)Cout * K;
+    const int wblocks = (int)((total / 4 + 191) / 192 > 4096 ? 4096 : (total / 4 + 191) / 192);
+    hipLaunchKernelGGL(wgrad_reduce_tm_kernel, dim3(wblocks + bblocks), dim3(192), 0, st, ws, dw_oihw, bslab, dbias,
+                       splits, Cout, total, accumulate, wblocks, bblocks);
   } else {
     const int wblocks = Cout * ((Cin + 63) / 64);
     hipLaunchKernelGGL(wgrad_reduce_kernel, dim3(wblocks + bblocks), dim3(192), 0, st, ws, dw_oihw, bslab, dbias,
@@ -2692,9 +2766,9 @@
   MDM_LAUNCH_STATUS();
 }
 
-extern "C" int mdm_pack_weight(const float* w_oihw, void* w_fwd, void* w_dgrad, int Cout, int Cin, int ksize,
-                               int Cin_pad, int Cout_pad, int kblock_fwd, int kblock_dgrad, int dtype,
-                               void* stream) {
+static int pack_weight_impl(const float* w_oihw, void* w_fwd, void* w_dgrad, int Cout, int Cin, int ksize,
+                            int Cin_pad, int Cout_pad, int kblock_fwd, int kblock_dgrad, int dtype, int src_tm,
+                            void* stream) {
   MDM_CHECK_ARG(w_oihw && w_fwd);
   MDM_CHECK_ARG(ksize == 1 || ksize == 3);
   MDM_CHECK_ARG(Cin_pad >= Cin && Cout_pad >= Cout);
@@ -2708,7 +2782,7 @@
     dim3 grid(Cin / 32, Cout / 32);
 #define MDM_PACK_TILED(TT, TAPS)                                                                               \
   hipLaunchKernelGGL((pack_weight_tiled_kernel<TT, TAPS>), grid, dim3(256), 0, st, w_oihw, (TT*)w_fwd, (TT*)w_dgrad, \
-                     Cout, Cin, kblock_fwd, kblock_dgrad)
+                     Cout, Cin, kblock_fwd, kblock_dgrad, src_tm)
     if (dtype == DT_F32) { if (taps == 9) MDM_PACK_TILED(float, 9); else MDM_PACK_TILED(float, 1); }
     else if (dtype == DT_BF16) { if (taps == 9) MDM_PACK_TILED(bf16, 9); else MDM_PACK_TILED(bf16, 1); }
     else MDM_CHECK_ARG(false);
@@ -2716,11 +2790,33 @@
     MDM_LAUNCH_STATUS();
   }
   if (dtype == DT_F32)
-    hipLaunchKernelGGL(pack_weight_kernel<float>, dim3(nb), dim3(256), 0, st, w_oihw, (float*)w_fwd, (float*)w_dgrad, Cout, Cin, taps, Cin_pad, Cout_pad, kblock_fwd, kblock_dgrad);
+    hipLaunchKernelGGL(pack_weight_kernel<float>, dim3(nb), dim3(256), 0, st, w_oihw, (float*)w_fwd, (float*)w_dgrad, Cout, Cin, taps, Cin_pad, Cout_pad, kblock_fwd, kblock_dgrad, src_tm);
   else if (dtype == DT_BF16)
-    hipLaunchKernelGGL(pack_weight_kernel<bf16>, dim3(nb), dim3(256), 0, st, w_oihw, (bf16*)w_fwd, (bf16*)w_dgrad, Cout, Cin, taps, Cin_pad, Cout_pad, kblock_fwd, kblock_dgrad);
+    hipLaunchKernelGGL(pack_weight_kernel<bf16>, dim3(nb), dim3(256), 0, st, w_oihw, (bf16*)w_fwd, (bf16*)w_dgrad, Cout, Cin, taps, Cin_pad, Cout_pad, kblock_fwd, kblock_dgrad, src_tm);
   else MDM_CHECK_ARG(false);
   MDM_LAUNCH_STATUS();
+}
+
+extern "C" int mdm_conv_wgrad_reduce(const float* ws, float* dw_oihw, float* dbias, const void* dy, int M, int Cin,
+                                     int Cout, int ksize, int accumulate, int dtype, void* stream) {
+  return wgrad_reduce_impl(ws, dw_oihw, dbias, dy, M, Cin, Cout, ksize, accumulate, dtype, 0, stream);
+}
+
+extern "C" int mdm_conv_wgrad_reduce_tm(const float* ws, float* dw_tm, float* dbias, const void* dy, int M, int Cin,
+                                        int Cout, int ksize, int accumulate, int dtype, void* stream) {
+  return wgrad_reduce_impl(ws, dw_tm, dbias, dy, M, Cin, Cout, ksize, accumulate, dtype, 1, stream);
+}
+
+extern "C" int mdm_pack_weight(const float* w_oihw, void* w_fwd, void* w_dgrad, int Cout, int Cin, int ksize,
+                               int Cin_pad, int Cout_pad, int kblock_fwd, int kblock_dgrad, int dtype,
+                               void* stream) {
+  return pack_weight_impl(w_oihw, w_fwd, w_dgrad, Cout, Cin, ksize, Cin_pad, Cout_pad, kblock_fwd, kblock_dgrad, dtype, 0, stream);
+}
+
+extern "C" int mdm_pack_weight_tm(const float* w_tm, void* w_fwd, void* w_dgrad, int Cout, int Cin, int ksize,
+                                  int Cin_pad, int Cout_pad, int kblock_fwd, int kblock_dgrad, int dtype,
+                                  void* stream) {
+  return pack_weight_impl(w_tm, w_fwd, w_dgrad, Cout, Cin, ksize, Cin_pad, Cout_pad, kblock_fwd, kblock_dgrad, dtype, 1, stream);
 }
 
 extern "C" int mdm_pack_weights_multi(const void* table, int n, int total_blocks, int dtype, void* stream) {
diff --git a/ml-mdm_amd/mdm_hip/distributed.py b/ml-mdm_amd/mdm_hip/distributed.py
--- a/ml-mdm_amd/mdm_hip/distributed.py
+++ b/ml-mdm_amd/mdm_hip/distributed.py
@@ -44,12 +44,36 @@
         dist.barrier()
 
 
+def tap_major_parameters(net):
+    if os.environ.get("MDM_HIP_ARENA_OIHW", "0") == "1":
+        return []
+    from .unet import ResNet
+
+    out = []
+    for m in net.modules():
+        if isinstance(m, ResNet):
+            for conv in (m.conv1, m.conv2):
+                w = conv.weight
+                if w.requires_grad and w.dim() == 4 and tuple(w.shape[2:]) == (3, 3) and tuple(conv.stride) == (1, 1) and w.shape[1] > 1:
+                    out.append(w)
+    return out
+
+
+def arena_view(flat, off, p, tap_major=False):
+    seg = flat[off:off + p.numel()]
+    if tap_major:
+        o, i, kh, kw = p.shape
+        return seg.view(o, kh, kw, i).permute(0, 3, 1, 2)
+    return seg.view_as(p)
+
+
 class GradReducer:
 
     def __init__(self, params, bucket_mb: float = 256.0, wire_dtype="auto", group=None, tail_mb: float = 8.0,
                  world_override: int = None, force_collectives: bool = False, head_mb: float = 64.0,
-                 record_timeline: bool = False, late_params=None):
+                 record_timeline: bool = False, late_params=None, tap_major=None):
         self.params = [p for p in params if p.requires_grad]
+        self._tap_major = {id(p) for p in (tap_major or [])}
         self.group = group
         self.nranks = dist.get_world_size(group) if dist.is_initialized() else 1
         if world_override is not None:
@@ -92,7 +116,7 @@
                 self.buckets.append((b_start, off))
                 b_start = off
             n = p.numel()
-            p.grad = self.flat[off:off + n].view_as(p)
+            p.grad = arena_view(self.flat, off, p, id(p) in self._tap_major)
             self._bucket_of[p] = len(self.buckets)
             off += n
             if off - b_start >= (head if not self.buckets else cap):
@@ -114,6 +138,9 @@
         if self.world > 1:
             for p in self.params:
                 p.register_post_accumulate_grad_hook(self._hook)
+
+    def is_tap_major(self, p):
+        return id(p) in self._tap_major
 
     def slot(self, p):
         ent = self._slots.get(p.data_ptr())
@@ -336,7 +363,7 @@
         late = net.late_gradient_parameters() if hasattr(net, "late_gradient_parameters") else None
         self.reducer = GradReducer(list(net.parameters()), bucket_mb=bucket_mb, wire_dtype=wire_dtype, tail_mb=tail_mb,
                                    force_collectives=force_collectives, head_mb=head_mb, record_timeline=record_timeline,
-                                   late_params=late)
+                                   late_params=late, tap_major=tap_major_parameters(net))
         self.reducer.broadcast_parameters(0)
 
     def forward(self, *args, **kwargs):
diff --git a/ml-mdm_amd/mdm_hip/ops.py b/ml-mdm_amd/mdm_hip/ops.py
--- a/ml-mdm_amd/mdm_hip/ops.py
+++ b/ml-mdm_amd/mdm_hip/ops.py
@@ -1,4 +1,5 @@
 import ctypes
+import os
 import weakref
 
 import torch
@@ -88,6 +89,11 @@
 
 def _c(t):
     return t if t is None or t.is_contiguous() else t.contiguous()
+
+
+def _tap_major(t):
+    return t is not None and t.dim() == 4 and t.shape[2] == 3 and t.shape[3] == 3 and not t.is_contiguous() \
+        and t.is_contiguous(memory_format=torch.channels_last)
 
 
 _wcache = {}
@@ -174,6 +180,7 @@
 
 _defer_wgrad = False
 _wgrad_queue = {}
+_GROUP3X3 = os.environ.get("MDM_HIP_GROUP3X3", "1") != "0"
 _WG_MAX = 32
 
 
@@ -197,8 +204,8 @@
                                                  _dt(xs[0]), _stream()), "mdm_conv_wgrad_grouped")
 
 
-def _queue_wgrad(x, dy, weight, bias, slot, bslot, M, cin, cout):
-    key = (M, cin, cout, x.device.index)
+def _queue_wgrad(x, dy, weight, bias, slot, bslot, M, cin, cout, geom=None):
+    key = (M, cin, cout, x.device.index) if geom is None else geom + (cin, cout, x.device.index)
     q = _wgrad_queue.setdefault(key, [])
     q.append((x, dy, weight, bias, slot, bslot))
     _sink_defer(weight)
@@ -212,31 +219,56 @@
     q = _wgrad_queue.pop(key, None)
     if not q:
         return
-    M, cin, cout, _ = key
+    geom = key[:3] if len(key) == 6 else None
+    if geom is None:
+        M, cin, cout, _ = key
+        N, H, W, ks = M, 1, 1, 1
+    else:
+        N, H, W, cin, cout, _ = key
+        M, ks = N * H * W, 3
     L = _lib.lib()
-    tile = ctypes.c_int(0)
-    _lib.check(L.mdm_conv_wgrad_group_plan(M, cout, cin, BF16, len(q), ctypes.byref(tile)), "mdm_conv_wgrad_group_plan")
+
+    def plan(n):
+        tile = ctypes.c_int(0)
+        _lib.check(L.mdm_conv_wgrad_group_plan(M, cout, ks * ks * cin, BF16, n, ctypes.byref(tile)), "mdm_conv_wgrad_group_plan")
+        return tile.value
+
     tensors = [t for e in q for t in (e[0], e[1])]
-    if tile.value and all((e[5] is not None) == (q[0][5] is not None) for e in q):
-        G = len(q)
-        arr = lambda vals: (ctypes.c_void_p * G)(*vals)
-        xs, dys, dws = arr([_p(e[0]) for e in q]), arr([_p(e[1]) for e in q]), arr([_p(e[4]) for e in q])
-        dbs = arr([_p(e[5]) for e in q]) if q[0][5] is not None else None
-
-        def go():
-            _prof_wrap("conv_wgrad grouped x%d M=%d N=%d K=%d" % (G, M, cout, cin), 2.0 * G * M * cout * cin, lambda: _lib.check(
-                L.mdm_conv_wgrad_grouped(xs, dys, dws, dbs, G, M, cin, cout, BF16, _stream()), "mdm_conv_wgrad_grouped"))
-            for e in q:
+    chunks, rest = [], list(q)
+    if all((e[5] is not None) == (q[0][5] is not None) for e in q):
+        if geom is None:
+            if plan(len(q)):
+                chunks, rest = [rest], []
+        else:
+            while len(rest) >= 2:
+                g = next((n for n in range(len(rest), 1, -1) if plan(n) == 256), 0)
+                if not g:
+                    break
+                chunks.append(rest[:g])
+                rest = rest[g:]
+
+    def go():
+        for c in chunks:
+            G = len(c)
+            arr = lambda vals: (ctypes.c_void_p * G)(*vals)
+            xs, dys, dws = arr([_p(e[0]) for e in c]), arr([_p(e[1]) for e in c]), arr([_p(e[4]) for e in c])
+            dbs = arr([_p(e[5]) for e in c]) if c[0][5] is not None else None
+            if geom is None:
+                _prof_wrap("conv_wgrad grouped x%d M=%d N=%d K=%d" % (G, M, cout, cin), 2.0 * G * M * cout * cin, lambda: _lib.check(
+                    L.mdm_conv_wgrad_grouped(xs, dys, dws, dbs, G, M, cin, cout, BF16, _stream()), "mdm_conv_wgrad_grouped"))
+            else:
+                _prof_wrap("conv_wgrad grouped 3x3 x%d M=%d N=%d K=%d" % (G, M, cout, 9 * cin), 2.0 * G * M * cout * 9 * cin,
+                           lambda: _lib.check(L.mdm_conv_wgrad_grouped3x3(xs, dys, dws, dbs, G, N, H, W, cin, cout, BF16, _stream()),
+                                              "mdm_conv_wgrad_grouped3x3"))
+            for e in c:
                 _grad_sink.ready(e[2])
                 if e[5] is not None:
                     _grad_sink.ready(e[3])
-    else:
-        def go():
-            for x, dy, w, b, slot, bslot in q:
-                _wgrad_launch(x, dy, M, 1, 1, cin, 1, 1, cout, 1, 1, out=slot, dbias=bslot)
-                _grad_sink.ready(w)
-                if bslot is not None:
-                    _grad_sink.ready(b)
+        for x, dy, w, b, slot, bslot in rest:
+            _wgrad_launch(x, dy, N, H, W, cin, H, W, cout, ks, 1, out=slot, dbias=bslot)
+            _grad_sink.ready(w)
+            if bslot is not None:
+                _grad_sink.ready(b)
 
     _off_critical_path(tensors, go)
 
@@ -312,6 +344,10 @@
     if _defer_wgrad and _async_wgrad and ks == 1 and x.dtype == torch.bfloat16 and M >= 4096:
         _queue_wgrad(x.reshape(M, cin), dy.reshape(M, cout), weight, bias, slot, bslot, M, cin, cout)
         return
+    if _defer_wgrad and _async_wgrad and _GROUP3X3 and ks == 3 and stride == 1 and x.dtype == torch.bfloat16 and M >= 4096 \
+            and Ho == H and Wo == W and not (H & (H - 1)) and not (W & (W - 1)) and _tap_major(slot) and slot.data_ptr() % 16 == 0:
+        _queue_wgrad(x, dy, weight, bias, slot, bslot, M, cin, cout, geom=(N, H, W))
+        return
 
     def go():
         _wgrad_launch(x, dy, N, H, W, cin, Ho, Wo, cout, ks, stride, out=slot, dbias=bslot)
@@ -348,7 +384,8 @@
     epv = 4 if dtype == torch.float32 else 8
     cin_pad, cout_pad = _round_up(cin, epv), _round_up(cout, epv)
     taps = ks * ks
-    w32 = _c(weight.detach().float())
+    tm = _tap_major(weight)
+    w32 = weight.detach().float() if tm else _c(weight.detach().float())
     need_d = cin_pad == cin and not forward_only
     prev = ent[key][1] if key in ent else None
     if prev is not None and prev[0].numel() == cout_pad * taps * cin_pad and prev[0].device == weight.device:
@@ -362,9 +399,9 @@
     kbf = bk if (ks == 3 and cin_pad % bk == 0) else 0
     kbd = bk if (ks == 3 and cout_pad % bk == 0) else 0
     _lib.check(
-        L.mdm_pack_weight(_p(w32), _p(wf), _p(wd), cout, cin, ks, cin_pad, cout_pad, kbf, kbd,
-                          F32 if dtype == torch.float32 else BF16, _stream()),
-        "mdm_pack_weight",
+        (L.mdm_pack_weight_tm if tm else L.mdm_pack_weight)(_p(w32), _p(wf), _p(wd), cout, cin, ks, cin_pad, cout_pad, kbf, kbd,
+                                                            F32 if dtype == torch.float32 else BF16, _stream()),
+        "mdm_pack_weight_tm" if tm else "mdm_pack_weight",
     )
     _repacked(wf, wd)
     bp = None
@@ -409,11 +446,14 @@
         ver, val = ent[dtype]
         wf, wd, bp, cin_pad, cout_pad, kbf, kbd = val
         cout, cin = w.shape[0], w.shape[1]
-        if cin_pad != cin or cout_pad != cout or cin % 32 or cout % 32 or w.dtype != torch.float32 or not w.is_contiguous():
+        tm = _tap_major(w)
+        if cin_pad != cin or cout_pad != cout or cin % 32 or cout % 32 or w.dtype != torch.float32 or not (w.is_contiguous() or tm):
             continue
         taps = w.shape[2] * w.shape[3] if w.dim() == 4 else 1
         if taps not in (1, 9):
             continue
+        if tm:
+            taps |= 0x100
         items.append((w, ent, ver, val, cout, cin, taps, kbf, kbd))
     if not items:
         return
@@ -560,6 +600,9 @@
     _lib.check(L.mdm_conv_wgrad_plan(M, Cout, K, _dt(x), ctypes.byref(splits), ctypes.byref(wsb)), "mdm_conv_wgrad_plan")
     ws = _f32_ws(wsb.value, x.device)
     dw = torch.empty((Cout, Cin, ks, ks), dtype=torch.float32, device=x.device) if out is None else out
+    tm = _tap_major(dw)
+    if not (tm or dw.is_contiguous()):
+        raise _lib.MdmHipError("weight-gradient destination is neither contiguous nor tap-major (strides %s)" % (tuple(dw.stride()),))
 
     def go():
         _lib.check(L.mdm_conv_wgrad(_p(x), _p(dy), 0 if dbias is None else 1, _p(ws), N, H, W, Cin, Ho, Wo, Cout, ks, stride,
@@ -575,8 +618,9 @@
         if _prof_shapes:
             name += " M=%d N=%d K=%d" % (M, Cout, K)
         _prof_wrap(name, 2.0 * M * Cout * K, go)
-    _lib.check(L.mdm_conv_wgrad_reduce(_p(ws), _p(dw), _p(dbias), _p(dy), M, Cin, Cout, ks, 0 if out is None else 1, _dt(x),
-                                       _stream()), "mdm_conv_wgrad_reduce")
+    _lib.check((L.mdm_conv_wgrad_reduce_tm if tm else L.mdm_conv_wgrad_reduce)(
+        _p(ws), _p(dw), _p(dbias), _p(dy), M, Cin, Cout, ks, 0 if out is None else 1, _dt(x), _stream()),
+        "mdm_conv_wgrad_reduce_tm" if tm else "mdm_conv_wgrad_reduce")
     return dw
 
 
diff --git a/ml-mdm_amd/mdm_hip/trainer.py b/ml-mdm_amd/mdm_hip/trainer.py
--- a/ml-mdm_amd/mdm_hip/trainer.py
+++ b/ml-mdm_amd/mdm_hip/trainer.py
@@ -5,7 +5,7 @@
 import torch
 
 from . import ops
-from .distributed import DataParallel, GradReducer
+from .distributed import DataParallel, GradReducer, arena_view, tap_major_parameters
 
 
 class FusedState:
@@ -15,7 +15,7 @@
         self.params = [p for p in net.parameters() if p.requires_grad]
         late = net.late_gradient_parameters() if hasattr(net, "late_gradient_parameters") else None
         self.reducer = reducer if reducer is not None else GradReducer(self.params, bucket_mb=bucket_mb, wire_dtype=wire_dtype,
-                                                                       late_params=late)
+                                                                       late_params=late, tap_major=tap_major_parameters(net))
         self.reducer.broadcast_parameters(0)
         flat = torch.empty_like(self.reducer.flat)
         self.slices = {}
@@ -23,8 +23,9 @@
         with torch.no_grad():
             for p in self.reducer.order:
                 n = p.numel()
-                flat[off:off + n].copy_(p.reshape(-1))
-                p.data = flat[off:off + n].view_as(p)
+                v = arena_view(flat, off, p, self.reducer.is_tap_major(p))
+                v.copy_(p)
+                p.data = v
                 self.slices[id(p)] = (off, n)
                 off += n
         self.flat_p = flat
@@ -46,7 +47,7 @@
 
     def view(self, arena, p):
         off, n = self.slices[id(p)]
-        return arena[off:off + n].view_as(p)
+        return arena_view(arena, off, p, self.reducer.is_tap_major(p))
 
     def finish_backward(self):
         ops.flush_wgrad_queue()
@@ -135,9 +136,16 @@
                 [(n, tuple(p.shape)) for n, p in ema_net.named_parameters()] != [(n, tuple(p.shape)) for n, p in net.named_parameters()]:
             return no("ModelEma on another device / of another shape / with persistent buffers")
     reducer = wrapped.reducer if isinstance(wrapped, DataParallel) else \
-        GradReducer(params, group=None, world_override=1)
+        GradReducer(params, group=None, world_override=1, tap_major=tap_major_parameters(net))
     if [id(p) for p in reducer.params] != [id(p) for p in params]:
         return no("the DataParallel wrapper's reducer does not hold exactly the vision model's parameters")
+    st = _install(net, params, optimizer, ema_net, reducer)
+    st.ema_id = id(ema_model) if ema_model is not None else None
+    optimizer._mdm_fused = st
+    return st
+
+
+def _install(net, params, optimizer, ema_net, reducer):
     had_state = {id(p): dict(optimizer.state.get(p, {})) for p in params}
     st = FusedState(net, reducer=reducer, use_ema=ema_net is not None, async_wgrad=os.environ.get("MDM_HIP_SERIAL_WGRAD", "0") != "1")
     with torch.no_grad():
@@ -179,8 +187,6 @@
                 ev = st.view(st.flat_ema, by_name[name])
                 ev.copy_(pe.detach())
                 pe.data = ev
-    st.ema_id = id(ema_model) if ema_model is not None else None
-    optimizer._mdm_fused = st
     return st
 
 
```

New measurement: 11.48 steps/s, median of 4. Within noise of the previous version (+0.2%).
